# jianglab/helicon

Measured on NVIDIA B200. Metric: denovo3D candidates/sec (solve+score), higher is better.
Workload: dtype f32 (u,v,h) / f64 (x,hbar; bounded branch), as scipy executes it

## Files before the change

helicon_b200/csrc/hb2_api.cu:

```cuda
#include "../../include/helicon_b200.h"
#include "hb2_kernels.cuh"
#include "hb2_trf.cuh"
#include "hb2_symm.cuh"
#include "hb2_tie.cuh"
#include "hb2_fwd_band.cuh"
#include "hb2_adj_tile.cuh"
#include "hb2_explicit.cuh"
#include "hb2_bilinear.cuh"

#include <cub/cub.cuh>
#include <nvtx3/nvToolsExt.h>

#include <algorithm>
#include <cstdio>
#include <cstring>
#include <cstdlib>
#include <string>
#include <vector>

struct NvtxRange {
  explicit NvtxRange(const char* name) { nvtxRangePushA(name); }
  ~NvtxRange() { nvtxRangePop(); }
  NvtxRange(const NvtxRange&) = delete;
  NvtxRange& operator=(const NvtxRange&) = delete;
// ... 1626 lines not shown
  b->created = true;
  return HB2_OK;
}

extern "C" int hb2_batch_set_pixel_masks(hb2_batch* b, int32_t n_masks, const uint8_t* masks, const int32_t* cand_mask) {
  if (!b || n_masks < 0 || (n_masks > 0 && !masks) || !cand_mask) return fail(HB2_ERR_ARG, "bad argument");
  if (!b->created) return fail(HB2_ERR_STATE, "hb2_batch_set_pixel_masks must follow hb2_batch_create");
  BD& B = b->B;
  CK(cudaSetDevice(b->P->device));
  cudaStream_t st = b->stream;
  const int nc = B.nc;
  const size_t npx = (size_t)B.L2 * B.D2;
  for (int c = 0; c < nc; ++c)
    if (cand_mask[c] >= n_masks) return fail(HB2_ERR_ARG, "cand_mask entry out of range");
  std::vector<uint8_t> hm(masks, masks + (size_t)n_masks * npx);
  std::vector<int> cm(cand_mask, cand_mask + nc);
  CK(upload(b->pool, &B.pixmask, hm, st));
  CK(upload(b->pool, &B.cand_pixmask, cm, st));
  if (n_masks == 0) B.pixmask = nullptr;
  std::vector<int> neg(nc, (int)0x80000000);
  CK(cudaMemcpyAsync(b->d_bmax, neg.data(), sizeof(int) * nc, cudaMemcpyHostToDevice, st));
  k_build_rhs<<<cdiv((long long)b->nviews * B.rows_per_view, 256), 256, 0, st>>>(B, b->P->d_pix, b->nviews, b->d_bmax);
  if (b->bilinear) k_bil_rhs<<<cdiv((long long)b->nviews * B.rows_per_view, 256), 256, 0, st>>>(B, b->P->d_pix, b->nviews, b->d_bmax);
  CKL();
  CK(cudaStreamSynchronize(st));
  return HB2_OK;
}

extern "C" void hb2_batch_destroy(hb2_batch* b) {
  if (!b) return;
  cudaSetDevice(b->P->device);
  cudaStreamSynchronize(b->stream);
  b->pool.free_all();
  for (cudaEvent_t e : b->ev_pool) cudaEventDestroy(e);
  if (b->side) { cudaStreamSynchronize(b->side); cudaStreamDestroy(b->side); }
  if (b->ev_fork) cudaEventDestroy(b->ev_fork);
  if (b->ev_join) cudaEventDestroy(b->ev_join);
  if (b->h_nactive) cudaFreeHost(b->h_nactive);
  delete b;
}

static int sym_ref_order(hb2_batch* b, int c, std::vector<int>& ord) {
  const int m = b->h_msym[c];
  ord.resize(m);
  for (int r = 0; r < m; ++r) ord[r] = r;
  if (m == 0 || !b->d_sym_g) return HB2_OK;
  std::vector<int> gref(m);
  CK(cudaMemcpyAsync(gref.data(), b->d_sym_g + b->h_symoff[c], sizeof(int) * m, cudaMemcpyDeviceToHost, b->stream));
  CK(cudaStreamSynchronize(b->stream));
  int start = 0;
  for (size_t rd = 0; rd < b->h_sym_round_end.size() && start < m; ++rd) {
    const int end = std::min(m, b->h_sym_round_end[rd][c]);
    if (end > start) std::sort(ord.begin() + start, ord.begin() + end, [&](int x, int y) { return gref[x] < gref[y]; });
    start = std::max(start, end);
  }
  return HB2_OK;
}

extern "C" int hb2_batch_sym_order(hb2_batch* b, int32_t c, int32_t* ord_host, int64_t capacity) {
  if (!b || !b->created || !ord_host || c < 0 || c >= b->B.nc) return fail(HB2_ERR_ARG, "bad argument");
  if (capacity < b->h_msym[c]) return fail(HB2_ERR_ARG, "capacity too small");
  CK(cudaSetDevice(b->P->device));
  std::vector<int> ord;
  if (int e = sym_ref_order(b, c, ord)) return e;
  memcpy(ord_host, ord.data(), sizeof(int) * ord.size());
  return HB2_OK;
}

extern "C" int hb2_batch_sym_rows(hb2_batch* b, int32_t c, int32_t* n_rows, int32_t* a_host, int32_t* b_host, int64_t capacity) {
  if (!b || !b->created || c < 0 || c >= b->B.nc) return fail(HB2_ERR_ARG, "bad argument");
  CK(cudaSetDevice(b->P->device));
  int m = b->h_msym[c];
  if (n_rows) *n_rows = m;
  if (a_host && b_host) {
    if (capacity < m) return fail(HB2_ERR_ARG, "capacity too small");
    CK(cudaMemcpyAsync(a_host, b->d_sym_a + b->h_symoff[c], sizeof(int) * m, cudaMemcpyDeviceToHost, b->stream));
    CK(cudaMemcpyAsync(b_host, b->d_sym_b + b->h_symoff[c], sizeof(int) * m, cudaMemcpyDeviceToHost, b->stream));
    const int L3P = b->B.L3P, nd = b->B.ndisk;
    const std::vector<int>& i2r = b->P->int2ref;
    std::vector<int> ord;
    if (int e = sym_ref_order(b, c, ord)) return e;
    std::vector<int> ta(a_host, a_host + m), tb(b_host, b_host + m);
    for (int r = 0; r < m; ++r) {
      a_host[r] = (ta[ord[r]] % L3P) * nd + i2r[ta[ord[r]] / L3P];
      b_host[r] = (tb[ord[r]] % L3P) * nd + i2r[tb[ord[r]] / L3P];
    }
  }
  return HB2_OK;
}

extern "C" int64_t hb2_batch_rows_padded(hb2_batch* b, int32_t c, int64_t* n_data_padded) {
  if (!b || !b->created || c < 0 || c >= b->B.nc) return fail(HB2_ERR_ARG, "bad argument");
  if (n_data_padded) *n_data_padded = b->h_mdata[c];
  return (int64_t)b->h_mdata[c] + b->h_msym[c];
}

extern "C" int hb2_batch_rhs(hb2_batch* b, int32_t c, float* out) {
  if (!b || !b->created || !out || c < 0 || c >= b->B.nc) return fail(HB2_ERR_ARG, "bad argument");
  CK(cudaSetDevice(b->P->device));
  CK(cudaMemcpyAsync(out, b->B.b + b->h_uoff[c], sizeof(float) * b->h_mdata[c], cudaMemcpyDeviceToHost, b->stream));
  CK(cudaStreamSynchronize(b->stream));
  return HB2_OK;
}

enum { KC_FWD_DATA = 0, KC_FWD_SYM = 1, KC_ADJ = 2, KC_UPDATE = 3, KC_SCALAR = 4, KC_NORM = 5, KC_N = 6 };
struct ProfScope {
  hb2_batch* b;
  cudaStream_t s;
  int first = 0;
  ProfScope(hb2_batch* b_, int cls, cudaStream_t s_ = nullptr) : b(b_), s(s_ ? s_ : b_->stream) {
    if (!b->profiling) return;
    while (b->ev_pool.size() < b->ev_next + 2) { cudaEvent_t e; cudaEventCreate(&e); b->ev_pool.push_back(e); }
    first = (int)b->ev_next;
    b->ev_used.push_back({cls, first});
    cudaEventRecord(b->ev_pool[first], s);
    b->ev_next += 2;
  }
  ~ProfScope() {
    if (!b->profiling) return;
    cudaEventRecord(b->ev_pool[first + 1], s);
  }
};

static void launch_fwd_data(hb2_batch* b, int mode) {
  ProfScope ps(b, KC_FWD_DATA);
  const BD& B = b->B;
  cudaStream_t st = b->stream;
  if (b->nviews == 0) return;
  if (b->n_tie_views > 0) {
    const float* src = mode == MODE_LSMR ? B.v : B.xs;
    if (b->bilinear) {
      const dim3 gv(b->n_tie_views, B.fwd_ppv);
#define FBIL(I, Q) k_fwd_bil<I, Q, float, false><<<gv, HB2_BLOCK, 0, st>>>(B, TD{}, src, B.u, mode)
#define FBILQ(I) do { if (B.L3P == 4) FBIL(I, 1); else if (B.L3P == 8) FBIL(I, 2); else if (B.L3P == 12) FBIL(I, 3); else FBIL(I, 4); } while (0)
      if (b->idx16) FBILQ(uint16_t); else FBILQ(uint32_t);
#undef FBILQ
#undef FBIL
      k_fwd_lsym<float, false><<<gv, HB2_BLOCK, 0, st>>>(B, TD{}, src, B.u, mode);
      b->extra_launches += 1;
    } else if (b->explicit_rows) k_fwd_csr<float, false><<<dim3(b->n_tie_views, B.fwd_ppv), HB2_BLOCK, 0, st>>>(B, TD{}, src, B.u, mode);
    else if (b->idx16) k_fwd_tie<uint16_t, float, false><<<dim3(b->n_tie_views, B.fwd_ppv), HB2_BLOCK, 0, st>>>(B, TD{}, src, B.u, mode);
    else k_fwd_tie<uint32_t, float, false><<<dim3(b->n_tie_views, B.fwd_ppv), HB2_BLOCK, 0, st>>>(B, TD{}, src, B.u, mode);
    b->extra_launches += 1;
  }
  if (B.fwd_band) {
    const size_t sm = b->fwd_band_smem;
    const dim3 gb(B.bt32.nband, B.nc), gr(b->max_views, B.nc);
#define FWB(Q)                                                                                            \
  do {                                                                                                    \
    hb2_allow_big_smem((const void*)k_fwd_band<Q, float, false>);                                         \
    k_fwd_band<Q, float, false><<<gb, HB2_FWDB_THREADS, sm, st>>>(B, TD{}, nullptr, mode);                \
    k_fwd_band_reduce<Q, float, false><<<gr, HB2_BLOCK, 0, st>>>(B, TD{}, nullptr, mode);                 \
  } while (0)
    if (B.L3P == 4) FWB(1); else if (B.L3P == 8) FWB(2); else if (B.L3P == 12) FWB(3); else FWB(4);
    b->extra_launches += 1;
#undef FWB
    return;
  }
  const int ntiles = (B.D2 + HB2_TILE_RAYS - 1) / HB2_TILE_RAYS;
  unsigned grid = (unsigned)b->nviews * ntiles;
#define FWD(T)                                                                              \
  do {                                                                                      \
    if (B.L3P == 4) k_fwd_data<T, 1><<<grid, HB2_BLOCK, 0, st>>>(B, mode);                  \
    else if (B.L3P == 8) k_fwd_data<T, 2><<<grid, HB2_BLOCK, 0, st>>>(B, mode);             \
    else if (B.L3P == 12) k_fwd_data<T, 3><<<grid, HB2_BLOCK, 0, st>>>(B, mode);            \
    else k_fwd_data<T, 4><<<grid, HB2_BLOCK, 0, st>>>(B, mode);                             \
  } while (0)
  if (b->idx16) FWD(uint16_t); else FWD(uint32_t);
#undef FWD
}
static void launch_fwd_sym(hb2_batch* b, int mode, cudaStream_t on = nullptr) {
  ProfScope ps(b, KC_FWD_SYM, on);
  const BD& B = b->B;
  dim3 g(B.part_us_per_cand, B.nc);
  k_fwd_sym<<<g, HB2_BLOCK, 0, on ? on : b->stream>>>(B, mode);
}
static void launch_adj(hb2_batch* b, int mode) {
  ProfScope ps(b, KC_ADJ);
  const BD& B = b->B;
  dim3 g(B.part_v_per_cand, B.nc);
  cudaStream_t st = b->stream;
  if (b->n_tie_views > 0) {
    if (b->bilinear) {
      const dim3 ga(cdiv(B.ndisk, (HB2_BLOCK / 32) * (32 / (B.L3P / 4))), B.nc);
      const size_t smt = (size_t)HB2_BILT_NS * HB2_BILT_SV * ((size_t)B.bil_KB * HB2_BLOCK * 6 + (size_t)B.bil_rmax * B.L3P * sizeof(float));
      const bool use_tile = B.bil_adj_tile && smt <= 200 * 1024;
#define ABIL(Q)                                                                                      \
  do {                                                                                               \
    k_bil_unblend<Q, float, false><<<b->n_tie_views, HB2_BLOCK, 0, st>>>(B, TD{}, B.u, B.bil_ub, mode); \
    if (use_tile && B.bil_KB == 3) {                                                                 \
      hb2_allow_big_smem((const void*)k_adj_bil_tile<Q, 3, float, false>);                           \
      k_adj_bil_tile<Q, 3, float, false><<<dim3(B.ntile, B.nc), HB2_BILT_THREADS, smt, st>>>(B, TD{}, B.bil_ub, B.vtie, mode); \
    } else if (use_tile) {                                                                           \
      hb2_allow_big_smem((const void*)k_adj_bil_tile<Q, 0, float, false>);                           \
      k_adj_bil_tile<Q, 0, float, false><<<dim3(B.ntile, B.nc), HB2_BILT_THREADS, smt, st>>>(B, TD{}, B.bil_ub, B.vtie, mode); \
    } else k_adj_bil<Q, float, false><<<ga, HB2_BLOCK, 0, st>>>(B, TD{}, B.bil_ub, B.vtie, mode);   \
  } while (0)
      if (B.L3P == 4) ABIL(1); else if (B.L3P == 8) ABIL(2); else if (B.L3P == 12) ABIL(3); else ABIL(4);
#undef ABIL
      k_adj_lsym<float, false><<<dim3(cdiv(B.npad, HB2_BLOCK), B.nc), HB2_BLOCK, 0, st>>>(B, TD{}, B.u, B.vtie, mode);
      b->extra_launches += 2;
    } else if (b->explicit_rows) k_adj_csc<float, false><<<dim3(cdiv(B.npad, HB2_BLOCK / 32), B.nc), HB2_BLOCK, 0, st>>>(B, TD{}, B.u, B.vtie, mode);
    else k_adj_tie<float, false><<<dim3(cdiv(B.ndisk, HB2_BLOCK), B.nc), HB2_BLOCK, 0, st>>>(B, TD{}, B.u, B.vtie, mode);
    b->extra_launches += 1;
  }
  if (B.adj_tile == 2) {
    const size_t sm = b->adj_tile_smem;
    const dim3 gc(B.ntile, B.nc, b->adj_chunks);
#define ADJTC(K)                                                                                                        \
  do {                                                                                                                  \
    hb2_allow_big_smem((const void*)k_adj_tile<4, K, float, false, true>);   \
    k_adj_tile<4, K, float, false, true><<<gc, HB2_ADJT_THREADS, sm, st>>>(B, TD{}, B.u, nullptr, mode);                \
  } while (0)
    if (B.K == 1) ADJTC(1); else ADJTC(2);
#undef ADJTC
    return;
  }
  if (B.adj_tile) {
    const size_t sm = b->adj_tile_smem;
#define ADJT(Q, K)                                                                                                   \
  do {                                                                                                               \
    hb2_allow_big_smem((const void*)k_adj_tile<Q, K, float, false>);      \
    k_adj_tile<Q, K, float, false><<<g, HB2_ADJT_THREADS, sm, st>>>(B, TD{}, B.u, nullptr, mode);                    \
  } while (0)
#define ADJTQ(K) do { if (B.L3P == 4) ADJT(1, K); else if (B.L3P == 8) ADJT(2, K); else if (B.L3P == 12) ADJT(3, K); else ADJT(4, K); } while (0)
    if (B.K == 1) ADJTQ(1); else ADJTQ(2);
#undef ADJTQ
#undef ADJT
    return;
  }
  if (B.adj_fast) {
    if (B.K == 1) k_adj_pq<1><<<g, HB2_BLOCK, 0, st>>>(B, mode);
    else k_adj_pq<2><<<g, HB2_BLOCK, 0, st>>>(B, mode);
    return;
  }
#define ADJ(K, M) k_adj<K, M><<<g, HB2_BLOCK, 0, st>>>(B, mode)
  if (B.MC == 1) ADJ(0, 1);
  else ADJ(0, 0);
#undef ADJ
}
static void launch_update(hb2_batch* b, int mode) {
  ProfScope ps(b, KC_UPDATE);
  const BD& B = b->B;
  dim3 g(B.part_x_per_cand, B.nc);
  k_update<<<g, HB2_BLOCK, 0, b->stream>>>(B, mode);
}

extern "C" int hb2_batch_apply_forward(hb2_batch* b, int32_t c, const float* x_host, float* y_host) {
  if (!b || !b->created || !x_host || !y_host || c < 0 || c >= b->B.nc) return fail(HB2_ERR_ARG, "bad argument");
  CK(cudaSetDevice(b->P->device));
  BD& B = b->B;
  cudaStream_t st = b->stream;
  long long m = (long long)b->h_mdata[c] + b->h_msym[c];
  std::vector<float> xi((size_t)B.npad, 0.f);
  for (int z = 0; z < B.L3; ++z)
    for (int pp = 0; pp < B.ndisk; ++pp) xi[(size_t)pp * B.L3P + z] = x_host[(size_t)z * B.ndisk + b->P->int2ref[pp]];
  CK(cudaMemcpyAsync(B.xs + (size_t)c * B.npad, xi.data(), sizeof(float) * B.npad, cudaMemcpyHostToDevice, st));
  CK(cudaMemsetAsync(B.u + b->h_uoff[c], 0, sizeof(float) * m, st));
  B.only_cand = c;
  launch_fwd_data(b, MODE_PLAIN);
  launch_fwd_sym(b, MODE_PLAIN);
  B.only_cand = -1;
  CKL();
  CK(cudaMemcpyAsync(y_host, B.u + b->h_uoff[c], sizeof(float) * m, cudaMemcpyDeviceToHost, st));
  CK(cudaStreamSynchronize(st));
  b->solved = false;
  return HB2_OK;
}

extern "C" int hb2_batch_apply_adjoint(hb2_batch* b, int32_t c, const float* y_host, float* x_host) {
  if (!b || !b->created || !x_host || !y_host || c < 0 || c >= b->B.nc) return fail(HB2_ERR_ARG, "bad argument");
  CK(cudaSetDevice(b->P->device));
  BD& B = b->B;
  cudaStream_t st = b->stream;
  long long m = (long long)b->h_mdata[c] + b->h_msym[c];
  CK(cudaMemcpyAsync(B.u + b->h_uoff[c], y_host, sizeof(float) * m, cudaMemcpyHostToDevice, st));
  B.only_cand = c;
  launch_adj(b, MODE_PLAIN);
  B.only_cand = -1;
  CKL();
  std::vector<float> xi((size_t)B.npad);
  CK(cudaMemcpyAsync(xi.data(), B.xs + (size_t)c * B.npad, sizeof(float) * B.npad, cudaMemcpyDeviceToHost, st));
  CK(cudaStreamSynchronize(st));
  for (int z = 0; z < B.L3; ++z)
    for (int pp = 0; pp < B.ndisk; ++pp) x_host[(size_t)z * B.ndisk + b->P->int2ref[pp]] = xi[(size_t)pp * B.L3P + z];
  b->solved = false;
  return HB2_OK;
}


static int run_trf(hb2_batch* b, const hb2_solve_options* opt, std::vector<TrfState>& out, long long& launches, int& outer_iters) {
  BD& B = b->B;
  cudaStream_t st = b->stream;
  const int nc = B.nc;
  bool any = false;
  for (int c = 0; c < nc; ++c) any = any || b->cands[c].positive;
  out.assign(nc, TrfState{});
  if (!any) return HB2_OK;
  DevPool tmp;
  tmp.owner = b;
  TD T{};
#define CKT2(call) do { cudaError_t e_ = (call); if (e_ != cudaSuccess) { tmp.free_all(); return fail(HB2_ERR_CUDA, std::string(#call) + ": " + cudaGetErrorString(e_)); } } while (0)
  const size_t nv = (size_t)nc * B.npad, nu = (size_t)b->u_total;
  double** nvecs[] = {&T.G, &T.D, &T.DH, &T.PH, &T.RH, &T.STEP, &T.V, &T.H, &T.HBAR, &T.XIN, &T.W, &T.UN};
  for (double** p : nvecs) CKT2(tmp.alloc(p, nv, true, st));
  B.vtie64 = nullptr;
  if (b->n_tie_views > 0) CKT2(tmp.alloc(&B.vtie64, nv, true, st));
  B.bil_ub64 = nullptr;
  if (b->bilinear) CKT2(tmp.alloc(&B.bil_ub64, nu, true, st));
  double** mvecs[] = {&T.R, &T.UM, &T.Y, &T.Y2};
  for (double** p : mvecs) CKT2(tmp.alloc(p, nu, true, st));
  long long max_m = 0;
  for (int c = 0; c < nc; ++c) max_m = std::max<long long>(max_m, (long long)b->h_mdata[c] + b->h_msym[c]);
  const unsigned gn = cdiv(B.npad, HB2_BLOCK * 4), gm = std::max(1u, cdiv(max_m, HB2_BLOCK * 4));
  T.red_slots = (int)std::max(gn, gm);
  CKT2(tmp.alloc(&T.red, (size_t)nc * T.red_slots * TRF_NRED, true, st));
  CKT2(tmp.alloc(&T.st, nc, true, st));
  CKT2(tmp.alloc(&T.nactive, 1, true, st));
  CKT2(tmp.alloc(&T.ninner, 1, true, st));
  {
    std::vector<float> bmax(nc);
    CKT2(cudaMemcpyAsync(bmax.data(), b->d_bmax, sizeof(float) * nc, cudaMemcpyDeviceToHost, st));
    CKT2(cudaStreamSynchronize(st));
    std::vector<TrfState> hs(nc, TrfState{});
    for (int c = 0; c < nc; ++c) {
      int iv;
      memcpy(&iv, &bmax[c], 4);
      iv = iv >= 0 ? iv : iv ^ 0x7fffffff;
      float ub;
      memcpy(&ub, &iv, 4);
      hs[c].needed = b->cands[c].positive ? 1 : 0;
      hs[c].lb = 0.0; hs[c].ub = (double)ub;
      hs[c].tol = opt->trf_tol > 0 ? opt->trf_tol : 1e-2;
      if (!(hs[c].ub > hs[c].lb)) hs[c].needed = 0;
    }
    CKT2(cudaMemcpyAsync(T.st, hs.data(), sizeof(TrfState) * nc, cudaMemcpyHostToDevice, st));
    CKT2(cudaStreamSynchronize(st));
  }
  const double EPS = 2.220446049250313e-16;
  const int lsmr_maxiter = opt->max_iter > 0 ? opt->max_iter : 1000;
  const int max_iter = opt->trf_max_iter > 0 ? opt->trf_max_iter : 200;
  const dim3 g_n(gn, nc), g_m(gm, nc), g_sym(std::max(1, B.part_us_per_cand), nc);
  const dim3 g_adj(cdiv((long long)B.ndisk * (B.L3P / 4), HB2_BLOCK), nc);
  const size_t sm64 = (size_t)HB2_ADJT_NS * HB2_ADJT_SV * B.K * HB2_BLOCK * sizeof(uint16_t) +
                      (size_t)HB2_ADJT_NS * HB2_ADJT_SV * B.rmax * B.L3P * sizeof(double);
  const unsigned g_fwd = (unsigned)b->nviews * ((B.D2 + HB2_TILE_RAYS - 1) / HB2_TILE_RAYS);
  const unsigned g_sc = cdiv(nc, 128);
  auto ew = [&](int op) { k_trf_ew<<<g_n, HB2_BLOCK, 0, st>>>(B, T, op); ++launches; };
  auto mw = [&](int op) { k_trf_mw<<<g_m, HB2_BLOCK, 0, st>>>(B, T, op); ++launches; };
  auto red = [&](int nslots, int add, int gate, int start = 0) { k_trf_reduce<<<nc, HB2_BLOCK, 0, st>>>(B, T, nslots, add, gate, start); ++launches; };
  auto sc = [&](int op) { k_trf_scal<<<g_sc, 128, 0, st>>>(B, T, op, EPS, lsmr_maxiter, max_iter); ++launches; };
  auto fwd = [&](const double* src, double* dst, int gate) {
    if (B.bt64.nband > 0) {
      const dim3 gb(B.bt64.nband, nc), gr(b->max_views, nc);
#define FWB64(Q)                                                                                          \
  do {                                                                                                    \
    hb2_allow_big_smem((const void*)k_fwd_band<Q, double, true>);                                         \
    k_fwd_band<Q, double, true><<<gb, HB2_FWDB_THREADS, b->fwd_band_smem64, st>>>(B, T, src, gate);       \
    k_fwd_band_reduce<Q, double, true><<<gr, HB2_BLOCK, 0, st>>>(B, T, dst, gate);                        \
  } while (0)
      if (B.L3P == 4) FWB64(2); else if (B.L3P == 8) FWB64(4); else if (B.L3P == 12) FWB64(6); else FWB64(8);
#undef FWB64
      ++launches;
    } else if (b->idx16) k_fwd64_data<uint16_t><<<g_fwd, HB2_BLOCK, 0, st>>>(B, T, src, dst, gate);
    else k_fwd64_data<uint32_t><<<g_fwd, HB2_BLOCK, 0, st>>>(B, T, src, dst, gate);
    k_fwd64_sym<<<g_sym, HB2_BLOCK, 0, st>>>(B, T, src, dst, gate);
    launches += 2;
    if (b->n_tie_views > 0) {
      if (b->bilinear) {
        const dim3 gv(b->n_tie_views, B.fwd_ppv);
#define FBIL(I, Q) k_fwd_bil<I, Q, double, true><<<gv, HB2_BLOCK, 0, st>>>(B, T, src, dst, gate)
#define FBILQ(I) do { if (B.L3P == 4) FBIL(I, 1); else if (B.L3P == 8) FBIL(I, 2); else if (B.L3P == 12) FBIL(I, 3); else FBIL(I, 4); } while (0)
        if (b->idx16) FBILQ(uint16_t); else FBILQ(uint32_t);
#undef FBILQ
#undef FBIL
        k_fwd_lsym<double, true><<<gv, HB2_BLOCK, 0, st>>>(B, T, src, dst, gate);
        ++launches;
      } else if (b->explicit_rows) k_fwd_csr<double, true><<<dim3(b->n_tie_views, B.fwd_ppv), HB2_BLOCK, 0, st>>>(B, T, src, dst, gate);
      else if (b->idx16) k_fwd_tie<uint16_t, double, true><<<dim3(b->n_tie_views, B.fwd_ppv), HB2_BLOCK, 0, st>>>(B, T, src, dst, gate);
      else k_fwd_tie<uint32_t, double, true><<<dim3(b->n_tie_views, B.fwd_ppv), HB2_BLOCK, 0, st>>>(B, T, src, dst, gate);
      ++launches;
    }
  };
  auto adj = [&](const double* rows, double* dst, int gate) {
    if (b->n_tie_views > 0) {
      if (b->bilinear) {
        const dim3 ga(cdiv(B.ndisk, (HB2_BLOCK / 32) * (32 / (B.L3P / 4))), nc);
        const size_t smt = (size_t)HB2_BILT_NS * HB2_BILT_SV * ((size_t)B.bil_KB * HB2_BLOCK * 6 + (size_t)B.bil_rmax * B.L3P * sizeof(double));
        const bool use_tile = B.bil_adj_tile && smt <= 200 * 1024;
#define ABIL(Q)                                                                                        \
  do {                                                                                                 \
    k_bil_unblend<Q, double, true><<<b->n_tie_views, HB2_BLOCK, 0, st>>>(B, T, rows, B.bil_ub64, gate); \
    if (use_tile) {                                                                                    \
      hb2_allow_big_smem((const void*)k_adj_bil_tile<Q, 0, double, true>);                             \
      k_adj_bil_tile<Q, 0, double, true><<<dim3(B.ntile, nc), HB2_BILT_THREADS, smt, st>>>(B, T, B.bil_ub64, B.vtie64, gate); \
    } else k_adj_bil<Q, double, true><<<ga, HB2_BLOCK, 0, st>>>(B, T, B.bil_ub64, B.vtie64, gate);    \
  } while (0)
        if (B.L3P == 4) ABIL(1); else if (B.L3P == 8) ABIL(2); else if (B.L3P == 12) ABIL(3); else ABIL(4);
#undef ABIL
        k_adj_lsym<double, true><<<dim3(cdiv(B.npad, HB2_BLOCK), nc), HB2_BLOCK, 0, st>>>(B, T, rows, B.vtie64, gate);
        launches += 2;
      } else if (b->explicit_rows) k_adj_csc<double, true><<<dim3(cdiv(B.npad, HB2_BLOCK / 32), nc), HB2_BLOCK, 0, st>>>(B, T, rows, B.vtie64, gate);
      else k_adj_tie<double, true><<<dim3(cdiv(B.ndisk, HB2_BLOCK), nc), HB2_BLOCK, 0, st>>>(B, T, rows, B.vtie64, gate);
      ++launches;
    }
    if (B.adj_tile == 1 && sm64 <= 200 * 1024) {
      const dim3 gt(B.ntile, nc);
#define ADJT64(Q, K)                                                                                                 \
  do {                                                                                                               \
    hb2_allow_big_smem((const void*)k_adj_tile<Q, K, double, true>);    \
    k_adj_tile<Q, K, double, true><<<gt, HB2_ADJT_THREADS, sm64, st>>>(B, T, rows, dst, gate);                       \
  } while (0)
#define ADJT64Q(K) do { if (B.L3P == 4) ADJT64(1, K); else if (B.L3P == 8) ADJT64(2, K); else if (B.L3P == 12) ADJT64(3, K); else ADJT64(4, K); } while (0)
      if (B.K == 1) ADJT64Q(1); else ADJT64Q(2);
#undef ADJT64Q
#undef ADJT64
    } else {
      k_adj64<<<g_adj, HB2_BLOCK, 0, st>>>(B, T, rows, dst, gate);
    }
    ++launches;
  };
  auto read_counter = [&](int* dptr, int& v) -> cudaError_t {
    cudaError_t e = cudaMemcpyAsync(b->h_nactive, dptr, sizeof(int), cudaMemcpyDeviceToHost, st);
    if (e != cudaSuccess) return e;
    e = cudaStreamSynchronize(st);
    v = *b->h_nactive;
    return e;
  };
  ew(EW_START); red(gn, 0, 0, 1); sc(SC_START);
  int nact = 0;
  CKT2(read_counter(T.nactive, nact));
  outer_iters = 0;
  if (nact > 0) {
    k_trf_start_apply<<<g_n, HB2_BLOCK, 0, st>>>(B, T); ++launches;
    fwd(T.W, T.Y, 0); mw(MW_RESID); red(gm, 0, 0); sc(SC_RESID0);
    adj(T.R, T.G, 0);
    for (int it = 0; it <= max_iter && nact > 0; ++it) {
      ew(EW_PREP); red(gn, 0, 0); sc(SC_PREP);
      CKT2(read_counter(T.nactive, nact));
      if (nact == 0) break;
      ++outer_iters;
      CKT2(cudaMemsetAsync(T.ninner, 0, sizeof(int), st));
      adj(T.UM, T.W, 0); ew(EW_INNER_INIT); red(gn, 0, 0); sc(SC_INNER_INIT);
      ew(EW_INNER_UPD);
      int ninner = 1;
      for (int k = 0; k < lsmr_maxiter && ninner > 0; ++k) {
        fwd(T.W, T.Y, 1); mw(MW_INNER_U); red(gm, 0, 1);
        ew(EW_INNER_UN); red(gn, 1, 1); sc(SC_INNER_BETA);
        adj(T.UM, T.W, 1); ew(EW_INNER_V); red(gn, 0, 1); sc(SC_INNER_ROT);
        ew(EW_INNER_UPD); red(gn, 0, 1); sc(SC_INNER_TEST);
        if (k % 2 == 1 || k + 1 == lsmr_maxiter) CKT2(read_counter(T.ninner, ninner));
      }
      ew(EW_STEP1); red(gn, 0, 0); sc(SC_STEP1);
      ew(EW_STEP2); red(gn, 0, 2); sc(SC_STEP2);
      fwd(T.W, T.Y, 2);
      ew(EW_LOAD_PH); fwd(T.W, T.Y2, 2);
      mw(MW_DOTS3); red(gm, 0, 2); sc(SC_SAVE_M);
      ew(EW_DOTS); red(gn, 0, 2); sc(SC_QUAD);
      ew(EW_AG); red(gn, 0, 2); sc(SC_SAVE_AG);
      fwd(T.W, T.Y, 2); mw(MW_DOT_YY); red(gm, 0, 2); sc(SC_AG);
      ew(EW_MKSTEP); red(gn, 0, 0); sc(SC_SAVE_SG);
      fwd(T.W, T.Y, 0); mw(MW_DOT_YY); red(gm, 0, 0); sc(SC_CC);
      ew(EW_XUPD);
      fwd(T.W, T.Y, 0); mw(MW_RESID); red(gm, 0, 0); sc(SC_RESID);
      adj(T.R, T.G, 0);
      CKT2(cudaGetLastError());
    }
  }
  ew(EW_FINAL);
  CKT2(cudaGetLastError());
  CKT2(cudaMemcpyAsync(out.data(), T.st, sizeof(TrfState) * nc, cudaMemcpyDeviceToHost, st));
  CKT2(cudaStreamSynchronize(st));
  tmp.free_all();
  B.vtie64 = nullptr;
  return HB2_OK;
}

extern "C" int hb2_batch_solve(hb2_batch* b, const hb2_solve_options* opt, hb2_result* res) {
  if (!b || !b->created || !opt || !res) return fail(HB2_ERR_ARG, "bad argument");
  CK(cudaSetDevice(b->P->device));
  NvtxRange nvtx_("solve_equations + score (batch)");
  nvtxRangePushA("solve_equations: LSMR");
  struct PopGuard { int n = 1; ~PopGuard() { while (n-- > 0) nvtxRangePop(); } } nvtx_stage_;
  BD& B = b->B;
  cudaStream_t st = b->stream;
  const int nc = B.nc;
  const int maxit = opt->max_iter > 0 ? opt->max_iter : 1000;
  const int check = opt->check_every > 0 ? opt->check_every : 8;
  B.clip_pred = opt->clip_pred;
  B.only_cand = -1;
  b->profiling = opt->profile != 0;
  b->ev_used.clear();
  b->ev_next = 0;
  cudaEvent_t e0, e1, e2;
  CK(cudaEventCreate(&e0)); CK(cudaEventCreate(&e1)); CK(cudaEventCreate(&e2));
  CK(cudaEventRecord(e0, st));
  size_t nv = (size_t)nc * B.npad;
  CK(cudaMemsetAsync(B.x, 0, nv * sizeof(double), st));
  CK(cudaMemsetAsync(B.hbar, 0, nv * sizeof(double), st));
  CK(cudaMemsetAsync(B.h, 0, nv * sizeof(float), st));
  CK(cudaMemsetAsync(B.v, 0, nv * sizeof(float), st));
  CK(cudaMemcpyAsync(B.u, B.b, sizeof(float) * (size_t)b->u_total, cudaMemcpyDeviceToDevice, st));
  CK(cudaMemsetAsync(b->d_nactive, 0, sizeof(int), st));
  long long launches = 0;
  b->extra_launches = 0;
  static const int env_norm = [] { const char* e = getenv("HB2_NORM_MODE"); return e ? atoi(e) : -1; }();
  const bool chain = (env_norm >= 0 ? env_norm : opt->norm_mode) != 0;
  if (chain) {
    hb2_allow_big_smem((const void*)k_chain_sumsq<CHAIN_U>);
    hb2_allow_big_smem((const void*)k_chain_sumsq<CHAIN_V>);
    hb2_allow_big_smem((const void*)k_chain_sumsq<CHAIN_B>);
  }
  float* ch_u = chain ? b->d_chain : nullptr;
  float* ch_v = chain ? b->d_chain + nc : nullptr;
  if (chain) { k_chain_sumsq<CHAIN_B><<<nc, 64, HB2_CHAIN_SMEM, st>>>(B, ch_u, MODE_INIT); ++launches; }
  k_scal_normb<<<nc, HB2_BLOCK, 0, st>>>(B, ch_u);
  launch_adj(b, MODE_INIT);
  if (chain) { k_chain_sumsq<CHAIN_V><<<nc, 64, HB2_CHAIN_SMEM, st>>>(B, ch_v, MODE_INIT); ++launches; }
  k_scal_init<<<nc, HB2_BLOCK, 0, st>>>(B, b->d_nactive, ch_v);
  launch_update(b, MODE_INIT);
  launches += 4;
  CKL();
  int it = 0;
  static const int env_overlap = [] { const char* e = getenv("HB2_OVERLAP"); return e ? atoi(e) : 1; }();
  const bool overlap = env_overlap != 0 && !b->profiling;
  if (overlap && !b->side) {
    CK(cudaStreamCreateWithFlags(&b->side, cudaStreamNonBlocking));
    CK(cudaEventCreateWithFlags(&b->ev_fork, cudaEventDisableTiming));
    CK(cudaEventCreateWithFlags(&b->ev_join, cudaEventDisableTiming));
  }
  *b->h_nactive = 1;
  CK(cudaMemcpyAsync(b->h_nactive, b->d_nactive, sizeof(int), cudaMemcpyDeviceToHost, st));
  CK(cudaStreamSynchronize(st));
  while (*b->h_nactive > 0 && it < maxit) {
    int burst = std::min(check, maxit - it);
    for (int q = 0; q < burst; ++q) {
      if (overlap) {
        cudaEventRecord(b->ev_fork, st);
        launch_fwd_data(b, MODE_LSMR);
        cudaStreamWaitEvent(b->side, b->ev_fork, 0);
        launch_fwd_sym(b, MODE_LSMR, b->side);
        cudaEventRecord(b->ev_join, b->side);
        cudaStreamWaitEvent(st, b->ev_join, 0);
      } else {
        launch_fwd_data(b, MODE_LSMR);
        launch_fwd_sym(b, MODE_LSMR);
      }
      if (chain) { ProfScope ps(b, KC_NORM); k_chain_sumsq<CHAIN_U><<<nc, 64, HB2_CHAIN_SMEM, st>>>(B, ch_u, MODE_LSMR); ++launches; }
      { ProfScope ps(b, KC_SCALAR); k_scal_beta<<<nc, HB2_BLOCK, 0, st>>>(B, ch_u); }
      launch_adj(b, MODE_LSMR);
      if (chain) { ProfScope ps(b, KC_NORM); k_chain_sumsq<CHAIN_V><<<nc, 64, HB2_CHAIN_SMEM, st>>>(B, ch_v, MODE_LSMR); ++launches; }
      { ProfScope ps(b, KC_SCALAR); k_scal_rot<<<nc, HB2_BLOCK, 0, st>>>(B, ch_v); }
      launch_update(b, MODE_LSMR);
      { ProfScope ps(b, KC_SCALAR); k_scal_test<<<nc, HB2_BLOCK, 0, st>>>(B, opt->atol, opt->btol, opt->conlim, maxit, opt->fixed_iters, b->d_nactive); }
      launches += 7;
    }
    it += burst;
    CKL();
    CK(cudaMemcpyAsync(b->h_nactive, b->d_nactive, sizeof(int), cudaMemcpyDeviceToHost, st));
    CK(cudaStreamSynchronize(st));
  }
  CK(cudaEventRecord(e1, st));
  std::vector<TrfState> trf;
  int trf_outer = 0;
  cudaEvent_t e1b;
  CK(cudaEventCreate(&e1b));
  {
    dim3 g(cdiv(B.npad, 256), nc);
    k_x_to_f32<<<g, 256, 0, st>>>(B);
    ++launches;
  }
  nvtxRangePop(); nvtxRangePushA("solve_equations: bounded TRF");
  if (opt->fixed_iters <= 0) {
    int rc = run_trf(b, opt, trf, launches, trf_outer);
    if (rc != HB2_OK) return rc;
  } else trf.assign(nc, TrfState{});
  CK(cudaEventRecord(e1b, st));
  nvtxRangePop(); nvtxRangePushA("cosine_similarity (reprojection + score)");
  {
    launch_fwd_data(b, MODE_SCORE);
    k_scal_score<<<nc, HB2_BLOCK, 0, st>>>(B, b->d_score);
    launches += 2;
    CKL();
  }
  CK(cudaEventRecord(e2, st));
  std::vector<LsmrState> hs(nc);
  std::vector<float> sc(nc);
  CK(cudaMemcpyAsync(hs.data(), B.st, sizeof(LsmrState) * nc, cudaMemcpyDeviceToHost, st));
  CK(cudaMemcpyAsync(sc.data(), b->d_score, sizeof(float) * nc, cudaMemcpyDeviceToHost, st));
  CK(cudaStreamSynchronize(st));
  float ms_l = 0, ms_s = 0, ms_t = 0;
  cudaEventElapsedTime(&ms_l, e0, e1); cudaEventElapsedTime(&ms_t, e1, e1b); cudaEventElapsedTime(&ms_s, e1b, e2);
  cudaEventDestroy(e0); cudaEventDestroy(e1); cudaEventDestroy(e1b); cudaEventDestroy(e2);
  for (double& t : b->timing) t = 0;
  b->timing[0] = ms_l; b->timing[1] = ms_t; b->timing[2] = ms_s; b->timing[13] = trf_outer; b->timing[3] = (double)(launches + b->extra_launches); b->timing[4] = it;
  if (b->profiling) {
    for (auto& pr : b->ev_used) {
      float ms = 0;
      cudaEventElapsedTime(&ms, b->ev_pool[pr.second], b->ev_pool[pr.second + 1]);
      if (pr.first == KC_NORM) b->timing[14] += ms;
      else b->timing[5 + pr.first] += ms;
      if (pr.first == KC_FWD_DATA) b->timing[10] += 1;
      if (pr.first == KC_ADJ) b->timing[11] += 1;
      if (pr.first == KC_UPDATE) b->timing[12] += 1;
    }
    b->profiling = false;
  }
  for (int c = 0; c < nc; ++c) {
    hb2_result& r = res[c];
    r.score = sc[c]; r.itn = hs[c].itn; r.istop = hs[c].istop; r.trf_nit = trf[c].status == 3 ? 0 : trf[c].nit;
    r.flags = b->cand_flags[c] | ((trf[c].needed && trf[c].status != 3) ? HB2_FLAG_BOUNDED : 0u);
    r.n_data_rows = 0; r.n_sym_rows = b->h_msym[c];
    r.normr = (float)hs[c].normr; r.normar = hs[c].normar; r.normA = (float)hs[c].normA; r.normx = (float)hs[c].normx;
  }
  b->solved = true;
  b->last_trf = trf;
  return HB2_OK;
}

extern "C" int hb2_batch_trf_trace(hb2_batch* b, int32_t c, double* out, int32_t max_rows) {
  if (!b || !out || c < 0 || c >= (int)b->last_trf.size()) return fail(HB2_ERR_ARG, "bad argument or no solve yet");
  const TrfState& S = b->last_trf[c];
  int n = std::min(std::min(S.nit, 24), (int)max_rows);
  for (int i = 0; i < n; ++i)
    for (int k = 0; k < 8; ++k) out[i * 8 + k] = S.trace[i][k];
  return S.nit * 16 + (S.status + 1);
}

extern "C" int hb2_batch_get_x(hb2_batch* b, int32_t c, float* x_host) {
  if (!b || !b->solved || !x_host || c < 0 || c >= b->B.nc) return fail(HB2_ERR_ARG, "bad argument or batch not solved");
  CK(cudaSetDevice(b->P->device));
  const BD& B = b->B;
  std::vector<float> xi((size_t)B.npad);
  CK(cudaMemcpyAsync(xi.data(), B.xs + (size_t)c * B.npad, sizeof(float) * B.npad, cudaMemcpyDeviceToHost, b->stream));
  CK(cudaStreamSynchronize(b->stream));
  for (int z = 0; z < B.L3; ++z)
    for (int pp = 0; pp < B.ndisk; ++pp) x_host[(size_t)z * B.ndisk + b->P->int2ref[pp]] = xi[(size_t)pp * B.L3P + z];
  return HB2_OK;
}

extern "C" int hb2_batch_timing(hb2_batch* b, double* out16) {
  if (!b || !out16) return fail(HB2_ERR_ARG, "null argument");
  memcpy(out16, b->timing, sizeof(b->timing));
  return HB2_OK;
}

extern "C" int hb2_lsmr_scalar_step(double* state64, int phase, float alpha, float beta, double normx, double atol,
                                    double btol, double conlim, int maxiter, float* coef_hbar, float* coef_x,
                                    float* coef_h, double* trace8) {
  static_assert(sizeof(LsmrState) <= 64 * sizeof(double), "state scratch too small");
  LsmrState S;
  memcpy(&S, state64, sizeof(S));
  int ret = 0;
  if (phase == 0) lsmr_init_(S, alpha, beta);
  else if (phase == 1) lsmr_rotate_(S, alpha, beta);
  else ret = lsmr_test_(S, normx, atol, btol, conlim, maxiter);
  memcpy(state64, &S, sizeof(S));
  if (coef_hbar) *coef_hbar = S.cf_hbar;
  if (coef_x) *coef_x = S.cf_x;
  if (coef_h) *coef_h = S.cf_h;
  if (trace8) {
    trace8[0] = S.rho; trace8[1] = S.rhobar; trace8[2] = S.zeta; trace8[3] = S.normr; trace8[4] = S.normA;
    trace8[5] = S.test1; trace8[6] = S.test2; trace8[7] = S.active;
  }
  return ret;
}

extern "C" int hb2_helical_symmetrize(const float* data_host, const hb2_symm_params* p, const int64_t* k_begin,
                                      const int32_t* ent_h, const int32_t* ent_floor, const int32_t* ent_ceil,
                                      const double* ent_wk, const double* mats, int32_t n_mats, float* vol_out_host,
                                      float* xsum_out, float* ysum_out, float* zsum_out, int device, void* stream) {
  NvtxRange nvtx_("apply_helical_symmetry");
  if (!data_host || !p || !k_begin || !mats) return fail(HB2_ERR_ARG, "null argument");
  if (hb2_device_count() <= 0) return fail(HB2_ERR_NO_DEVICE, "no CUDA device visible; helicon_b200 has no CPU fallback");
  if (p->nz1 <= 0 || p->ny1 <= 0 || p->nx1 <= 0 || p->csym <= 0 || p->n_ent < 0) return fail(HB2_ERR_ARG, "bad sizes");
  if (p->zs0 < 0 || p->zs1 > p->nz1) return fail(HB2_ERR_ARG, "z-section slab outside the output");
  CK(cudaSetDevice(device));
  cudaStream_t st = (cudaStream_t)stream;
  SymmP P{};
  P.nz0 = p->nz0; P.ny0 = p->ny0; P.nx0 = p->nx0; P.nz = p->nz; P.ny = p->ny; P.nx = p->nx;
  P.oz = p->oz; P.oy = p->oy; P.ox = p->ox; P.nz1 = p->nz1; P.ny1 = p->ny1; P.nx1 = p->nx1;
  P.apix = p->apix; P.new_apix = p->new_apix; P.csym = p->csym; P.zs0 = p->zs0; P.zs1 = p->zs1;
  for (int e = 0; e < p->n_ent; ++e)
    if (ent_floor[e] < 0 || ent_ceil[e] >= p->nz0 || ent_h[e] < 0 || (long long)(ent_h[e] + 1) * p->csym > n_mats)
      return fail(HB2_ERR_ARG, "entry table out of range");
  DevPool pool;
  const size_t nd = (size_t)p->nz0 * p->ny0 * p->nx0, nv = (size_t)p->nz1 * p->ny1 * p->nx1;
  float *d_data, *d_vol, *d_x, *d_y, *d_z;
  long long* d_kb; int *d_h, *d_f, *d_c; double *d_w, *d_m;
#define CKS(call) do { cudaError_t e_ = (call); if (e_ != cudaSuccess) { pool.free_all(); return fail(HB2_ERR_CUDA, std::string(#call) + ": " + cudaGetErrorString(e_)); } } while (0)
  CKS(pool.alloc(&d_data, nd, false, st)); CKS(pool.alloc(&d_vol, nv, false, st));
  CKS(pool.alloc(&d_x, (size_t)p->nz1 * p->ny1, false, st)); CKS(pool.alloc(&d_y, (size_t)p->nz1 * p->nx1, false, st));
  CKS(pool.alloc(&d_z, (size_t)p->ny1 * p->nx1, false, st));
  CKS(pool.alloc(&d_kb, (size_t)p->nz1 + 1, false, st)); CKS(pool.alloc(&d_h, (size_t)p->n_ent, false, st));
  CKS(pool.alloc(&d_f, (size_t)p->n_ent, false, st)); CKS(pool.alloc(&d_c, (size_t)p->n_ent, false, st));
  CKS(pool.alloc(&d_w, (size_t)p->n_ent, false, st)); CKS(pool.alloc(&d_m, (size_t)n_mats * 4, false, st));
  CKS(cudaMemcpyAsync(d_data, data_host, nd * sizeof(float), cudaMemcpyHostToDevice, st));
  CKS(cudaMemcpyAsync(d_kb, k_begin, ((size_t)p->nz1 + 1) * sizeof(long long), cudaMemcpyHostToDevice, st));
  if (p->n_ent) {
    CKS(cudaMemcpyAsync(d_h, ent_h, (size_t)p->n_ent * sizeof(int), cudaMemcpyHostToDevice, st));
    CKS(cudaMemcpyAsync(d_f, ent_floor, (size_t)p->n_ent * sizeof(int), cudaMemcpyHostToDevice, st));
    CKS(cudaMemcpyAsync(d_c, ent_ceil, (size_t)p->n_ent * sizeof(int), cudaMemcpyHostToDevice, st));
    CKS(cudaMemcpyAsync(d_w, ent_wk, (size_t)p->n_ent * sizeof(double), cudaMemcpyHostToDevice, st));
  }
  CKS(cudaMemcpyAsync(d_m, mats, (size_t)n_mats * 4 * sizeof(double), cudaMemcpyHostToDevice, st));
  k_symm_volume<<<cdiv((long long)nv, 256), 256, 0, st>>>(P, d_data, d_kb, d_h, d_f, d_c, d_w, d_m, d_vol);
  const long long nproj = (long long)p->nz1 * p->ny1 + (long long)p->nz1 * p->nx1 + (long long)p->ny1 * p->nx1;
  k_symm_project<<<cdiv(nproj, 128), 128, 0, st>>>(P, d_vol, d_x, d_y, d_z);
  CKS(cudaGetLastError());
  if (vol_out_host) CKS(cudaMemcpyAsync(vol_out_host, d_vol, nv * sizeof(float), cudaMemcpyDeviceToHost, st));
  if (xsum_out) CKS(cudaMemcpyAsync(xsum_out, d_x, (size_t)p->nz1 * p->ny1 * sizeof(float), cudaMemcpyDeviceToHost, st));
  if (ysum_out) CKS(cudaMemcpyAsync(ysum_out, d_y, (size_t)p->nz1 * p->nx1 * sizeof(float), cudaMemcpyDeviceToHost, st));
  if (zsum_out) CKS(cudaMemcpyAsync(zsum_out, d_z, (size_t)p->ny1 * p->nx1 * sizeof(float), cudaMemcpyDeviceToHost, st));
  CKS(cudaStreamSynchronize(st));
  pool.free_all();
#undef CKS
  return HB2_OK;
}

struct hb2_scoremap {
  int device = 0;
  long long n = 0;
  float* d_score = nullptr;
  int* d_itn = nullptr;
  unsigned* d_flags = nullptr;
  long long* d_idx = nullptr;
  size_t idx_cap = 0;
  float* d_top = nullptr;
  long long* d_topi = nullptr;
  int top_cap = 0;
};

__global__ void k_scoremap_fill(float* __restrict__ sc, int* __restrict__ it, unsigned* __restrict__ fl, long long n) {
  const long long i = (long long)blockIdx.x * blockDim.x + threadIdx.x;
  if (i < n) { sc[i] = __int_as_float(0x7fc00000); it[i] = 0; fl[i] = 0u; }
}
__global__ void k_scoremap_scatter(const float* __restrict__ score, const LsmrState* __restrict__ st,
                                   const long long* __restrict__ idx, int nc, long long n, float* __restrict__ sc,
                                   int* __restrict__ it, unsigned* __restrict__ fl) {
  const int c = blockIdx.x * blockDim.x + threadIdx.x;
  if (c >= nc) return;
  const long long t = idx[c];
  if (t < 0 || t >= n) return;
  sc[t] = score[c];
  it[t] = st[c].itn;
  fl[t] = (unsigned)idx[nc + c];
}
__global__ void k_scoremap_merge(float* __restrict__ sc, int* __restrict__ it, unsigned* __restrict__ fl,
                                 const float* __restrict__ g, int n_maps, long long n) {
  const long long i = (long long)blockIdx.x * blockDim.x + threadIdx.x;
  if (i >= n) return;
  float s = sc[i];
  int q = it[i];
  unsigned f = fl[i];
  for (int r = 0; r < n_maps; ++r) {
    const float v = g[(size_t)r * 3 * n + i];
    if (v == v && !(s == s)) {
      s = v;
      q = reinterpret_cast<const int*>(g)[(size_t)r * 3 * n + n + i];
      f = reinterpret_cast<const unsigned*>(g)[(size_t)r * 3 * n + 2 * n + i];
    }
  }
  sc[i] = s; it[i] = q; fl[i] = f;
}
__global__ void __launch_bounds__(1024) k_scoremap_topk(const float* __restrict__ sc, long long n, int k,
                                                        float* __restrict__ top, long long* __restrict__ topi) {
  __shared__ float s_v[32];
  __shared__ long long s_i[32];
  __shared__ float prev_v;
  __shared__ long long prev_i;
  if (threadIdx.x == 0) { prev_v = INFINITY; prev_i = -1; }
  __syncthreads();
// ... 156 lines not shown
```

helicon_b200/csrc/hb2_trf.cuh:

```cuda
#pragma once
#include "hb2_kernels.cuh"

#define TRF_NRED 8

struct Lsmr64 {
  double alpha, beta, normb;
  double zetabar, alphabar, rho, rhobar, cbar, sbar;
  double betadd, betad, rhodold, tautildeold, thetatilde, zeta, d;
  double normA2, maxrbar, minrbar, normA, normr, normar, normx, condA, rhotemp;
  double cf_hbar, cf_x, cf_h, inv_alpha, inv_beta;
  int minrbar_inf, itn, istop, active, skip_adj;
};

struct TrfState {
  double lb, ub, tol;
  double cost, g_norm, theta, lsmr_tol, p_dot_g, p_stride, r_stride_u, r_stride_l, r_stride, ag_stride;
  double cost_change;
  double coef_p, coef_r, coef_ag;
  double acc[TRF_NRED];
  double m0, m1, m2, r_value, p_value, ag_n0, ag_n1, ag_min, step_g;
  int active;
  int needed;
  int status, nit, stop_next, full_step;
  Lsmr64 in;
  double ag_value;
  double trace[24][8];
};

struct TD {
  TrfState* st;
  double *G, *D, *DH, *PH, *RH, *STEP, *V, *H, *HBAR, *XIN, *W, *UN;
  double *R, *UM, *Y, *Y2;
  double* red;
  int red_slots;
  int* nactive;
  int* ninner;
};

HB2_HD void sym_ortho64_(double a, double b, double& c, double& s, double& r) {
  if (b == 0.0) { c = a > 0 ? 1.0 : (a < 0 ? -1.0 : 0.0); s = 0.0; r = fabs(a); }
  else if (a == 0.0) { c = 0.0; s = b > 0 ? 1.0 : -1.0; r = fabs(b); }
  else if (fabs(b) > fabs(a)) { double tau = a / b; s = (b > 0 ? 1.0 : -1.0) / sqrt(1 + tau * tau); c = s * tau; r = b / s; }
  else { double tau = b / a; c = (a > 0 ? 1.0 : -1.0) / sqrt(1 + tau * tau); s = c * tau; r = a / c; }
}
HB2_HD void lsmr64_init_(Lsmr64& S, double alpha, double beta) {
  S.alpha = alpha; S.beta = beta; S.normb = beta;
  S.zetabar = alpha * beta; S.alphabar = alpha; S.rho = 1; S.rhobar = 1; S.cbar = 1; S.sbar = 0;
  S.betadd = beta; S.betad = 0; S.rhodold = 1; S.tautildeold = 0; S.thetatilde = 0; S.zeta = 0; S.d = 0;
  S.normA2 = alpha * alpha; S.maxrbar = 0; S.minrbar = 0; S.minrbar_inf = 1; S.normA = sqrt(S.normA2);
  S.condA = 1; S.normx = 0; S.normr = beta; S.normar = alpha * beta; S.itn = 0; S.istop = 0; S.skip_adj = 0;
  S.cf_hbar = S.cf_x = S.cf_h = 0; S.rhotemp = 0;
  S.inv_alpha = alpha > 0 ? 1.0 / alpha : 1.0;
  S.inv_beta = beta > 0 ? 1.0 / beta : 0.0;
  S.active = (S.normar != 0.0 && beta != 0.0) ? 1 : 0;
}
HB2_HD void lsmr64_rotate_(Lsmr64& S, double alpha, double beta) {
  S.itn += 1; S.alpha = alpha; S.beta = beta;
  double chat = S.alphabar > 0 ? 1.0 : (S.alphabar < 0 ? -1.0 : 0.0), alphahat = fabs(S.alphabar);
  double rhoold = S.rho, c, s;
  sym_ortho64_(alphahat, beta, c, s, S.rho);
  double thetanew = s * alpha;
  S.alphabar = c * alpha;
  double rhobarold = S.rhobar, zetaold = S.zeta, thetabar = S.sbar * S.rho;
  S.rhotemp = S.cbar * S.rho;
  double cb, sb, rb;
  sym_ortho64_(S.cbar * S.rho, thetanew, cb, sb, rb);
  S.cbar = cb; S.sbar = sb; S.rhobar = rb;
  S.zeta = S.cbar * S.zetabar; S.zetabar = -S.sbar * S.zetabar;
  S.cf_hbar = -(thetabar * S.rho / (rhoold * rhobarold));
  S.cf_x = S.zeta / (S.rho * S.rhobar);
  S.cf_h = -(thetanew / S.rho);
  double betaacute = chat * S.betadd, betahat = c * betaacute;
  S.betadd = -s * betaacute;
  double thetatildeold = S.thetatilde, ct, st, rt;
  sym_ortho64_(S.rhodold, thetabar, ct, st, rt);
  S.thetatilde = st * S.rhobar; S.rhodold = ct * S.rhobar;
  S.betad = -st * S.betad + ct * betahat;
  S.tautildeold = (zetaold - thetatildeold * S.tautildeold) / rt;
  double taud = (S.zeta - S.thetatilde * S.tautildeold) / S.rhodold;
  S.normr = sqrt(S.d + (S.betad - taud) * (S.betad - taud) + S.betadd * S.betadd);
  S.normA2 += beta * beta; S.normA = sqrt(S.normA2); S.normA2 += alpha * alpha;
  S.maxrbar = fmax(S.maxrbar, rhobarold);
  if (S.itn > 1) { S.minrbar = S.minrbar_inf ? rhobarold : fmin(S.minrbar, rhobarold); S.minrbar_inf = 0; }
  double mn = S.minrbar_inf ? S.rhotemp : fmin(S.minrbar, S.rhotemp);
  S.condA = fmax(S.maxrbar, S.rhotemp) / mn;
  S.normar = fabs(S.zetabar);
  S.inv_alpha = alpha > 0 ? 1.0 / alpha : 1.0;
}
HB2_HD int lsmr64_test_(Lsmr64& S, double normx, double atol, double btol, double conlim, int maxiter) {
  S.normx = normx;
  double test1 = S.normr / S.normb;
  double test2 = (S.normA * S.normr) != 0 ? S.normar / (S.normA * S.normr) : INFINITY;
  double test3 = 1 / S.condA;
  double t1 = test1 / (1 + S.normA * normx / S.normb);
  double rtol = btol + atol * S.normA * normx / S.normb;
  double ctol = conlim > 0 ? 1 / conlim : 0;
  int istop = 0;
  if (S.itn >= maxiter) istop = 7;
  if (1 + test3 <= 1) istop = 6;
  if (1 + test2 <= 1) istop = 5;
  if (1 + t1 <= 1) istop = 4;
  if (test3 <= ctol) istop = 3;
  if (test2 <= atol) istop = 2;
  if (test1 <= rtol) istop = 1;
  S.istop = istop;
  return istop;
}

__device__ __forceinline__ bool trf_gate(const TrfState& S, int gate) {
  if (!S.active) return false;
  if (gate == 1) return S.in.active != 0;
  if (gate == 2) return S.full_step == 0;
  return true;
}

template <typename IdxT>
__global__ void __launch_bounds__(HB2_BLOCK) k_fwd64_data(BD B, TD T, const double* __restrict__ src, double* __restrict__ dst,
                                                         int inner) {
  const int ntiles = (B.D2 + HB2_TILE_RAYS - 1) / HB2_TILE_RAYS;
  const int view = blockIdx.x / ntiles, tile = blockIdx.x % ntiles;
  const int c = B.view_cand[view];
  if (B.view_tie && B.view_tie[view] >= 0) return;
  const TrfState& S = T.st[c];
  if (!trf_gate(S, inner)) return;
  __shared__ int s_colk[HB2_MAX_ZMC];
  for (int e = threadIdx.x; e < B.ZMC; e += HB2_BLOCK) s_colk[e] = B.colk[B.view_colbegin[view] + e];
  __syncthreads();
  const int a = B.view_angle[view];
  const int D2 = B.D2, L3 = B.L3, L3P = B.L3P, MC = B.MC, ZMP = B.ZMP;
  const IdxT* __restrict__ fm = (const IdxT*)B.fmap + (size_t)a * D2 * D2;
  const double* __restrict__ vsrc = src + (size_t)c * B.npad;
  double* urow = dst + B.view_uoff[view];
  const int warp = threadIdx.x >> 5, lane = threadIdx.x & 31;
  const int q = lane & 3, sg = lane >> 2;
  const uint8_t* __restrict__ pm = cand_mask(B, c);
  for (int r = warp; r < HB2_TILE_RAYS; r += HB2_BLOCK / 32) {
    const int j = tile * HB2_TILE_RAYS + r;
    if (j >= D2) break;
    if (!B.rayvalid[a * D2 + j]) continue;
    const IdxT* __restrict__ fj = fm + (size_t)j * D2;
    for (int z0 = 0; z0 < L3P; z0 += 16) {
      double acc[4] = {0, 0, 0, 0};
      const int zq = z0 + 4 * q;
      if (zq < L3P) {
        const double* __restrict__ vb = vsrc + zq;
        for (int i0 = sg; i0 < D2; i0 += 32) {
          IdxT ids[4];
#pragma unroll
          for (int w = 0; w < 4; ++w) ids[w] = (i0 + 8 * w < D2) ? fj[i0 + 8 * w] : Sent<IdxT>::v;
          double2 ta[4], tb[4];
#pragma unroll
          for (int w = 0; w < 4; ++w) {
            if (ids[w] != Sent<IdxT>::v) {
              const double2* vp = reinterpret_cast<const double2*>(vb + (size_t)ids[w] * L3P);
              ta[w] = __ldg(vp); tb[w] = __ldg(vp + 1);
            } else {
              ta[w] = make_double2(0.0, 0.0); tb[w] = make_double2(0.0, 0.0);
            }
          }
#pragma unroll
          for (int w = 0; w < 4; ++w)
            if (ids[w] != Sent<IdxT>::v) { acc[0] += ta[w].x; acc[1] += ta[w].y; acc[2] += tb[w].x; acc[3] += tb[w].y; }
        }
      }
#pragma unroll
      for (int o = 4; o < 32; o <<= 1)
#pragma unroll
        for (int t = 0; t < 4; ++t) acc[t] += __shfl_xor_sync(0xffffffffu, acc[t], o);
      if (sg < 4) {
        const int z = zq + sg;
        if (z < L3) {
          const double sum = sg == 0 ? acc[0] : (sg == 1 ? acc[1] : (sg == 2 ? acc[2] : acc[3]));
          for (int mc = 0; mc < MC; ++mc) {
            const int zm = z * MC + mc;
            if (s_colk[zm] >= 0 && !(pm && !pm[(size_t)s_colk[zm] * D2 + j])) urow[(size_t)j * ZMP + zm] = sum;
          }
        }
      }
    }
  }
}

__global__ void __launch_bounds__(HB2_BLOCK) k_fwd64_sym(BD B, TD T, const double* __restrict__ src, double* __restrict__ dst,
                                                        int inner) {
  const int c = blockIdx.y;
  const TrfState& S = T.st[c];
  if (!trf_gate(S, inner)) return;
  const int m = B.cand_msym[c];
  const double* __restrict__ vsrc = src + (size_t)c * B.npad;
  double* us = dst + B.cand_uoff[c] + B.cand_mdata[c];
  const int* __restrict__ sa = B.sym_a + B.cand_symoff[c];
  const int* __restrict__ sb = B.sym_b + B.cand_symoff[c];
  for (int r = blockIdx.x * HB2_BLOCK * 4 + threadIdx.x, qq = 0; qq < 4; ++qq, r += HB2_BLOCK)
    if (r < m) us[r] = __ldg(vsrc + sa[r]) - __ldg(vsrc + sb[r]);
}

__global__ void __launch_bounds__(HB2_BLOCK) k_adj64(BD B, TD T, const double* __restrict__ rows, double* __restrict__ dst,
                                                    int inner) {
  const int c = blockIdx.y;
  const TrfState& S = T.st[c];
  if (!trf_gate(S, inner) || (inner == 1 && S.in.skip_adj)) return;
  const int L3 = B.L3, L3P = B.L3P, ZMP = B.ZMP, ndisk = B.ndisk, K = B.K, MC = B.MC;
  const int NQ = L3P >> 2;
  const int t = blockIdx.x * HB2_BLOCK + threadIdx.x;
  const int p = t / NQ, q = t - p * NQ;
  if (p >= ndisk) return;
  const int slot = B.aslot[p];
  const int z0 = 4 * q;
  double acc[4] = {0.0, 0.0, 0.0, 0.0};
  const int vb = B.cand_view_begin[c], nv = B.cand_view_count[c];
  for (int vi = 0; vi < nv; ++vi) {
    const int view = vb + vi;
    if (B.view_tie && B.view_tie[view] >= 0) continue;
    const int a = __ldg(B.view_angle + view);
    const double* __restrict__ ub = rows + __ldg(B.view_uoff + view) + z0 * MC;
    const uint16_t* __restrict__ am = B.amap + (size_t)a * K * B.apitch + slot;
    for (int k = 0; k < K; ++k) {
      const uint16_t j = am[(size_t)k * B.apitch];
      if (j != 0xFFFFu) {
        const double* __restrict__ uj = ub + (size_t)j * ZMP;
        if (MC == 1) {
          const double2 r0 = __ldg(reinterpret_cast<const double2*>(uj));
          const double2 r1 = __ldg(reinterpret_cast<const double2*>(uj) + 1);
          acc[0] += r0.x; acc[1] += r0.y; acc[2] += r1.x; acc[3] += r1.y;
        } else {
#pragma unroll
          for (int zz = 0; zz < 4; ++zz)
            if (z0 + zz < L3)
              for (int mc = 0; mc < MC; ++mc) acc[zz] += __ldg(uj + zz * MC + mc);
        }
      }
    }
  }
  const int* __restrict__ ptr = B.csc_ptr + (size_t)c * (B.npad + 1);
  const int* __restrict__ ent = B.csc_ent + B.cand_cscoff[c];
  const double* __restrict__ us = rows + B.cand_uoff[c] + B.cand_mdata[c];
  double* vdst = dst + (size_t)c * B.npad + (size_t)p * L3P + z0;
  if (B.vtie64 && B.cand_tie_count[c] > 0) {
    const double* vt = B.vtie64 + (size_t)c * B.npad + (size_t)p * L3P + z0;
#pragma unroll
    for (int zz = 0; zz < 4; ++zz) acc[zz] += vt[zz];
  }
#pragma unroll
  for (int zz = 0; zz < 4; ++zz) {
    double a2 = acc[zz];
    if (z0 + zz < L3) {
      const int g = p * L3P + z0 + zz;
      for (int e = ptr[g]; e < ptr[g + 1]; ++e) {
        int en = ent[e];
        double val = __ldg(us + (en & 0x7fffffff));
        a2 += en < 0 ? -val : val;
      }
    }
    vdst[zz] = a2;
  }
}

__device__ __forceinline__ double block_minmax_d(double x, bool is_min, double* shd) {
#pragma unroll
  for (int o = 16; o > 0; o >>= 1) {
    double y = __shfl_xor_sync(0xffffffffu, x, o);
    x = is_min ? fmin(x, y) : fmax(x, y);
  }
  int w = threadIdx.x >> 5, l = threadIdx.x & 31;
  if (l == 0) shd[w] = x;
  __syncthreads();
  if (w == 0) {
    x = l < HB2_BLOCK / 32 ? shd[l] : (is_min ? INFINITY : -INFINITY);
#pragma unroll
    for (int o = 16; o > 0; o >>= 1) {
      double y = __shfl_xor_sync(0xffffffffu, x, o);
      x = is_min ? fmin(x, y) : fmax(x, y);
    }
  }
  __syncthreads();
  return x;
}
__device__ __forceinline__ void trf_store_partials(TD T, int c, int slot, double (&v)[TRF_NRED], double* shd) {
#pragma unroll
  for (int k = 0; k < TRF_NRED; ++k) {
    double x = k < 6 ? block_sum_d(v[k], shd) : block_minmax_d(v[k], k == 6, shd);
    if (threadIdx.x == 0) T.red[((size_t)c * T.red_slots + slot) * TRF_NRED + k] = x;
  }
}
__global__ void __launch_bounds__(HB2_BLOCK) k_trf_reduce(BD B, TD T, int nslots, int add, int gate, int start) {
  const int c = blockIdx.x;
  __shared__ double shd[HB2_BLOCK / 32];
  TrfState& S = T.st[c];
  if (!(start ? (S.needed != 0) : trf_gate(S, gate))) return;
  double v[TRF_NRED];
#pragma unroll
  for (int k = 0; k < TRF_NRED; ++k) v[k] = k < 6 ? 0.0 : (k == 6 ? INFINITY : -INFINITY);
  for (int s2 = threadIdx.x; s2 < nslots; s2 += HB2_BLOCK) {
    const double* p = T.red + ((size_t)c * T.red_slots + s2) * TRF_NRED;
#pragma unroll
    for (int k = 0; k < 6; ++k) v[k] += p[k];
    v[6] = fmin(v[6], p[6]); v[7] = fmax(v[7], p[7]);
  }
#pragma unroll
  for (int k = 0; k < TRF_NRED; ++k) {
    double x = k < 6 ? block_sum_d(v[k], shd) : block_minmax_d(v[k], k == 6, shd);
    if (threadIdx.x == 0) {
      if (add) S.acc[k] = k < 6 ? S.acc[k] + x : (k == 6 ? fmin(S.acc[k], x) : fmax(S.acc[k], x));
      else S.acc[k] = x;
    }
  }
}

__device__ __forceinline__ double step_to_bound(double x, double s, double lb, double ub) {
  if (s == 0.0) return INFINITY;
  return fmax((lb - x) / s, (ub - x) / s);
}

enum {
  EW_START = 0,
  EW_PREP,
  EW_INNER_INIT,
  EW_INNER_UN,
  EW_INNER_V,
  EW_INNER_UPD,
  EW_STEP1,
  EW_STEP2,
  EW_LOAD_PH,
  EW_DOTS,
  EW_AG,
  EW_MKSTEP,
  EW_XUPD,
  EW_FINAL
};

__global__ void __launch_bounds__(HB2_BLOCK) k_trf_ew(BD B, TD T, int op) {
  const int c = blockIdx.y;
  __shared__ double shd[HB2_BLOCK / 32];
  const TrfState& S = T.st[c];
  bool act;
  if (op == EW_START || op == EW_FINAL) act = S.needed != 0;
  else if (op == EW_INNER_UPD) act = S.active && (S.in.active || S.in.itn == 0);
  else if (op == EW_INNER_UN || op == EW_INNER_V) act = trf_gate(S, 1);
  else if (op == EW_STEP2 || op == EW_LOAD_PH || op == EW_DOTS || op == EW_AG) act = trf_gate(S, 2);
  else act = trf_gate(S, 0);
  if (op == EW_INNER_V && S.in.skip_adj) act = false;
  if (!act) return;
  const size_t o = (size_t)c * B.npad;
  double* X = B.x + o;
  double red[TRF_NRED] = {0, 0, 0, 0, 0, 0, INFINITY, -INFINITY};
  const double lb = S.lb, ub = S.ub;
  for (int i = blockIdx.x * HB2_BLOCK * 4 + threadIdx.x, qq = 0; qq < 4; ++qq, i += HB2_BLOCK) {
    if (i >= B.npad || (i % B.L3P) >= B.L3) continue;
    const size_t e = o + i;
    switch (op) {
      case EW_START: {
        double y = X[i];
        red[6] = fmin(red[6], y); red[7] = fmax(red[7], y);
      } break;
      case EW_PREP: {
        double x = X[i], g = T.G[e], v = 1.0, dv = 0.0;
        if (g < 0) { v = ub - x; dv = -1.0; }
        if (g > 0) { v = x - lb; dv = 1.0; }
        T.D[e] = sqrt(v); T.DH[e] = g * dv;
        red[7] = fmax(red[7], fabs(g * v));
      } break;
      case EW_INNER_INIT: {
        double vt = T.D[e] * T.W[e];
        T.UN[e] = 0.0; T.V[e] = vt; red[0] += vt * vt;
      } break;
      case EW_INNER_UN: {
        double un = sqrt(T.DH[e]) * T.V[e] - S.in.alpha * (T.UN[e] * S.in.inv_beta);
        T.UN[e] = un; red[0] += un * un;
      } break;
      case EW_INNER_V: {
        double vt = (T.D[e] * T.W[e] + sqrt(T.DH[e]) * T.UN[e]) * S.in.inv_beta - S.in.beta * T.V[e];
        T.V[e] = vt; red[0] += vt * vt;
      } break;
      case EW_INNER_UPD: {
        double vn = T.V[e];
        if (S.in.itn == 0 || !S.in.skip_adj) { vn *= S.in.inv_alpha; T.V[e] = vn; }
        if (S.in.itn == 0) { T.H[e] = vn; T.HBAR[e] = 0.0; T.XIN[e] = 0.0; }
        else {
          double ho = T.H[e];
          double hb = T.HBAR[e] * S.in.cf_hbar + ho;
          T.HBAR[e] = hb;
          double xn = T.XIN[e] + S.in.cf_x * hb;
          T.XIN[e] = xn;
          T.H[e] = ho * S.in.cf_h + vn;
          red[0] += xn * xn;
        }
        T.W[e] = T.D[e] * vn;
      } break;
      case EW_STEP1: {
        double ph = -T.XIN[e];
        T.PH[e] = ph;
        double x = X[i], p = T.D[e] * ph, xp = x + p;
        red[6] = fmin(red[6], fmin(xp - lb, ub - xp));
        red[5] += p * T.G[e];
        red[7] = fmax(red[7], -step_to_bound(x, p, lb, ub));
      } break;
      case EW_STEP2: {
        double ph = T.PH[e], x = X[i], d = T.D[e];
        double p = d * ph;
        double st = step_to_bound(x, p, lb, ub);
        double rh = (st == S.p_stride && p != 0.0) ? -ph : ph;
        T.RH[e] = rh;
        T.PH[e] = ph * S.p_stride;
        double xb = x + p * S.p_stride, r = d * rh;
        red[7] = fmax(red[7], -step_to_bound(xb, r, lb, ub));
        T.W[e] = r;
      } break;
      case EW_LOAD_PH: T.W[e] = T.D[e] * T.PH[e]; break;
      case EW_DOTS: {
        double ph = T.PH[e], rh = T.RH[e], dh = T.DH[e], gh = T.D[e] * T.G[e];
        red[0] += rh * dh * rh; red[1] += gh * rh; red[2] += ph * dh * rh; red[3] += gh * ph; red[4] += ph * dh * ph;
      } break;
      case EW_AG: {
        double d = T.D[e], g = T.G[e], gh = d * g, agh = -gh, ag = d * agh;
        red[0] += agh * T.DH[e] * agh; red[1] += gh * agh;
        red[7] = fmax(red[7], -step_to_bound(X[i], ag, lb, ub));
        T.W[e] = ag;
      } break;
      case EW_MKSTEP: {
        double d = T.D[e];
        double s2 = d * (S.coef_p * T.PH[e] + S.coef_r * T.RH[e] - S.coef_ag * (d * T.G[e]));
        T.STEP[e] = s2; T.W[e] = s2; red[0] += s2 * T.G[e];
      } break;
      case EW_XUPD: {
        double x = X[i];
        if (S.cost_change >= 0) {
          x = x + T.STEP[e];
          if (x <= lb) x = nextafter(lb, ub);
          if (x >= ub) x = nextafter(ub, lb);
          if (x < lb || x > ub) x = 0.5 * (lb + ub);
          X[i] = x;
        }
        T.W[e] = x;
      } break;
      case EW_FINAL: B.xs[e] = (float)X[i]; break;
    }
  }
  if (op == EW_LOAD_PH || op == EW_XUPD || op == EW_FINAL) return;
  trf_store_partials(T, c, blockIdx.x, red, shd);
}

__global__ void __launch_bounds__(HB2_BLOCK) k_trf_start_apply(BD B, TD T) {
  const int c = blockIdx.y;
  const TrfState& S = T.st[c];
  if (!S.active) return;
  double* X = B.x + (size_t)c * B.npad;
  const double lb = S.lb, ub = S.ub, d = ub - lb;
  for (int i = blockIdx.x * HB2_BLOCK * 4 + threadIdx.x, qq = 0; qq < 4; ++qq, i += HB2_BLOCK) {
    if (i >= B.npad || (i % B.L3P) >= B.L3) continue;
    double y = X[i];
    double t = fmod(y - lb, 2 * d);
    if (t < 0) t += 2 * d;
    double x = lb + fmin(t, 2 * d - t);
    double ld = x - lb, udist = ub - x;
    double lth = 0.1 * fmax(1.0, fabs(lb)), uth = 0.1 * fmax(1.0, fabs(ub));
    bool la = ld <= fmin(udist, lth), ua = udist <= fmin(ld, uth);
    if (la) x = lb + 0.1 * fmax(1.0, fabs(lb));
    if (ua) x = ub - 0.1 * fmax(1.0, fabs(ub));
    if (x < lb || x > ub) x = 0.5 * (lb + ub);
    X[i] = x;
    T.W[(size_t)c * B.npad + i] = x;
  }
}

enum { MW_RESID = 0, MW_INNER_U, MW_DOTS3, MW_DOT_YY };
__global__ void __launch_bounds__(HB2_BLOCK) k_trf_mw(BD B, TD T, int op) {
  const int c = blockIdx.y;
  __shared__ double shd[HB2_BLOCK / 32];
  const TrfState& S = T.st[c];
  bool act = op == MW_INNER_U ? trf_gate(S, 1) : (op == MW_DOTS3 ? trf_gate(S, 2) : trf_gate(S, 0));
  if (!act) return;
  const long long m = (long long)B.cand_mdata[c] + B.cand_msym[c];
  const size_t o = (size_t)B.cand_uoff[c];
  double red[TRF_NRED] = {0, 0, 0, 0, 0, 0, INFINITY, -INFINITY};
  for (long long r = (long long)blockIdx.x * HB2_BLOCK * 4 + threadIdx.x, qq = 0; qq < 4; ++qq, r += HB2_BLOCK) {
    if (r >= m) continue;
    const size_t e = o + r;
    switch (op) {
      case MW_RESID: {
        double bb = r < B.cand_mdata[c] ? (double)B.b[e] : 0.0;
        double res = T.Y[e] - bb;
        T.R[e] = res; T.UM[e] = res; red[0] += res * res;
      } break;
      case MW_INNER_U: {
        double un = T.Y[e] - S.in.alpha * (T.UM[e] * S.in.inv_beta);
        T.UM[e] = un; red[0] += un * un;
      } break;
      case MW_DOTS3: {
        double v1 = T.Y[e], u1 = T.Y2[e];
        red[0] += v1 * v1; red[1] += u1 * v1; red[2] += u1 * u1;
      } break;
      case MW_DOT_YY: { double v = T.Y[e]; red[0] += v * v; } break;
    }
  }
  trf_store_partials(T, c, blockIdx.x, red, shd);
}

enum {
  SC_START = 0, SC_RESID0, SC_PREP, SC_INNER_INIT, SC_INNER_BETA, SC_INNER_ROT, SC_INNER_TEST, SC_STEP1, SC_STEP2,
  SC_SAVE_M, SC_QUAD, SC_SAVE_AG, SC_AG, SC_SAVE_SG, SC_CC, SC_RESID
};
__device__ __forceinline__ void min_quadratic_1d(double a, double b, double lo, double hi, double c, double& t, double& y) {
  double tt[3] = {lo, hi, 0};
  int n = 2;
  if (a != 0) {
    double ext = -0.5 * b / a;
    if (lo < ext && ext < hi) tt[n++] = ext;
  }
  t = tt[0]; y = tt[0] * (a * tt[0] + b) + c;
  for (int k = 1; k < n; ++k) {
    double yy = tt[k] * (a * tt[k] + b) + c;
    if (yy < y) { y = yy; t = tt[k]; }
  }
}
__global__ void k_trf_scal(BD B, TD T, int op, double eps, int lsmr_maxiter, int max_iter) {
  const int c = blockIdx.x * blockDim.x + threadIdx.x;
  if (c >= B.nc) return;
  TrfState& S = T.st[c];
  if (op == SC_START) { if (!S.needed) return; }
  else if (op == SC_INNER_BETA || op == SC_INNER_ROT || op == SC_INNER_TEST) { if (!trf_gate(S, 1)) return; }
  else if (op == SC_STEP2 || op == SC_SAVE_M || op == SC_QUAD || op == SC_SAVE_AG || op == SC_AG) { if (!trf_gate(S, 2)) return; }
  else if (!trf_gate(S, 0)) return;
  const double* r = S.acc;
  switch (op) {
    case SC_START: {
      bool inb = r[6] >= S.lb && r[7] <= S.ub;
      S.active = inb ? 0 : 1; S.status = inb ? 3 : 0; S.nit = 0; S.stop_next = 0; S.full_step = 0;
      if (!inb) atomicAdd(T.nactive, 1);
    } break;
    case SC_RESID0: S.cost = 0.5 * r[0]; break;
    case SC_PREP: {
      S.g_norm = r[7];
      bool stop = S.stop_next != 0;
      if (S.g_norm < S.tol) { S.status = 1; stop = true; }
      if (!stop && S.nit >= max_iter) stop = true;
      if (stop) { S.active = 0; if (S.nit < max_iter) S.nit += 1; atomicSub(T.nactive, 1); break; }
      S.nit += 1;
      if (S.nit <= 24) { S.trace[S.nit - 1][0] = S.cost; S.trace[S.nit - 1][1] = S.g_norm; }
      double eta = 1e-2 * fmin(0.5, S.g_norm);
      S.lsmr_tol = fmax(eps, fmin(0.1, eta * S.g_norm));
      S.theta = 1 - fmin(0.005, S.g_norm);
      S.in.beta = sqrt(2 * S.cost);
      S.in.inv_beta = S.in.beta > 0 ? 1.0 / S.in.beta : 0.0;
      S.in.itn = 0; S.in.active = 1; S.in.skip_adj = 0; S.in.alpha = 0; S.full_step = 0;
    } break;
    case SC_INNER_INIT: {
      double nv = sqrt(r[0]);
      double beta = S.in.beta;
      lsmr64_init_(S.in, nv * (beta > 0 ? 1.0 / beta : 0.0), beta);
      S.in.inv_alpha = nv > 0 ? 1.0 / nv : 1.0;
      if (S.in.active) atomicAdd(T.ninner, 1);
    } break;
    case SC_INNER_BETA: {
      S.in.beta = sqrt(r[0]);
      if (S.in.beta > 0) { S.in.inv_beta = 1.0 / S.in.beta; S.in.skip_adj = 0; } else S.in.skip_adj = 1;
    } break;
    case SC_INNER_ROT: lsmr64_rotate_(S.in, S.in.skip_adj ? S.in.alpha : sqrt(r[0]), S.in.beta); break;
    case SC_INNER_TEST: {
      int istop = lsmr64_test_(S.in, sqrt(r[0]), S.lsmr_tol, S.lsmr_tol, 1e8, lsmr_maxiter);
      if (istop > 0) { S.in.active = 0; atomicSub(T.ninner, 1); }
    } break;
    case SC_STEP1: {
      S.p_dot_g = r[5];
      if (S.p_dot_g > 0) { S.status = -1; S.stop_next = 1; }
      S.full_step = r[6] >= 0.0 ? 1 : 0;
      S.p_stride = -r[7];
      if (S.full_step) { S.coef_p = 1.0; S.coef_r = 0.0; S.coef_ag = 0.0; }
    } break;
    case SC_STEP2: {
      double rsu = -r[7];
      S.r_stride_l = (1 - S.theta) * rsu;
      S.r_stride_u = rsu * S.theta;
    } break;
    case SC_SAVE_M: S.m0 = r[0]; S.m1 = r[1]; S.m2 = r[2]; break;
    case SC_QUAD: {
      double a = 0.5 * (S.m0 + r[0]);
      double b = r[1] + S.m1 + r[2];
      double cc = 0.5 * S.m2 + r[3] + 0.5 * r[4];
      if (S.r_stride_u > 0) min_quadratic_1d(a, b, S.r_stride_l, S.r_stride_u, cc, S.r_stride, S.r_value);
      else { S.r_value = INFINITY; S.r_stride = 0; }
      double th = S.theta;
      S.p_value = 0.5 * (th * th * S.m2 + th * th * r[4]) + th * r[3];
    } break;
    case SC_SAVE_AG: S.ag_n0 = r[0]; S.ag_n1 = r[1]; S.ag_min = -r[7]; break;
    case SC_AG: {
      double a = 0.5 * (r[0] + S.ag_n0), b = S.ag_n1;
      double ag_value;
      min_quadratic_1d(a, b, 0.0, S.ag_min * S.theta, 0.0, S.ag_stride, ag_value);
      S.ag_value = ag_value;
      if (S.p_value < S.r_value && S.p_value < ag_value) { S.coef_p = S.theta; S.coef_r = 0; S.coef_ag = 0; }
      else if (S.r_value < S.p_value && S.r_value < ag_value) { S.coef_p = 1.0; S.coef_r = S.r_stride; S.coef_ag = 0; }
      else { S.coef_p = 0; S.coef_r = 0; S.coef_ag = S.ag_stride; }
    } break;
    case SC_SAVE_SG: S.step_g = r[0]; break;
    case SC_CC: {
      S.cost_change = -(0.5 * r[0] + S.step_g);
      if (S.nit <= 24) {
        double* t = S.trace[S.nit - 1];
        t[2] = S.in.itn;
        t[3] = S.full_step ? 0 : (S.coef_ag != 0 ? 3 : (S.coef_r != 0 ? 2 : 1));
        t[4] = S.p_value; t[5] = S.r_value; t[6] = S.ag_value; t[7] = S.cost_change;
      }
    } break;
    case SC_RESID: {
      if (S.cost_change < S.tol * S.cost) { S.status = 2; S.stop_next = 1; }
      S.cost = 0.5 * r[0];
    } break;
  }
}
```

Before: 54.46.

## Fuse TRF elementwise, reduce and scalar kernels; batch step-selection forward passes

Replaces the separate elementwise, m-space, reduce and scalar-update kernels of the bounded TRF solver with templated per-op pass kernels and a reduce kernel that also performs the scalar state update. Several outer-iteration phases are merged so the three candidate-step forward projections (p, r, anti-gradient) run back to back into separate buffers. This removes many small launches and redundant forward and adjoint applications per iteration. Each thread now handles more elements, reductions are masked to the needed slots, and the adjoint at inner-loop initialisation is dropped. The cost is extra m-space buffers and a more intricate op/mask table that must stay numerically equivalent to the previous sequence. A profiling script is added alongside.

```diff
diff --git a/helicon_b200/csrc/hb2_api.cu b/helicon_b200/csrc/hb2_api.cu
--- a/helicon_b200/csrc/hb2_api.cu
+++ b/helicon_b200/csrc/hb2_api.cu
@@ -1952,18 +1952,20 @@
   TD T{};
 #define CKT2(call) do { cudaError_t e_ = (call); if (e_ != cudaSuccess) { tmp.free_all(); return fail(HB2_ERR_CUDA, std::string(#call) + ": " + cudaGetErrorString(e_)); } } while (0)
   const size_t nv = (size_t)nc * B.npad, nu = (size_t)b->u_total;
-  double** nvecs[] = {&T.G, &T.D, &T.DH, &T.PH, &T.RH, &T.STEP, &T.V, &T.H, &T.HBAR, &T.XIN, &T.W, &T.UN};
+  double** nvecs[] = {&T.G, &T.D, &T.DH, &T.PH, &T.RH, &T.V, &T.H, &T.HBAR, &T.XIN, &T.W, &T.UN};
   for (double** p : nvecs) CKT2(tmp.alloc(p, nv, true, st));
+  T.W2 = T.HBAR; T.AG = T.H;
   B.vtie64 = nullptr;
   if (b->n_tie_views > 0) CKT2(tmp.alloc(&B.vtie64, nv, true, st));
   B.bil_ub64 = nullptr;
   if (b->bilinear) CKT2(tmp.alloc(&B.bil_ub64, nu, true, st));
-  double** mvecs[] = {&T.R, &T.UM, &T.Y, &T.Y2};
+  double** mvecs[] = {&T.R, &T.UM, &T.Y, &T.YP, &T.YAG};
   for (double** p : mvecs) CKT2(tmp.alloc(p, nu, true, st));
   long long max_m = 0;
   for (int c = 0; c < nc; ++c) max_m = std::max<long long>(max_m, (long long)b->h_mdata[c] + b->h_msym[c]);
-  const unsigned gn = cdiv(B.npad, HB2_BLOCK * 4), gm = std::max(1u, cdiv(max_m, HB2_BLOCK * 4));
-  T.red_slots = (int)std::max(gn, gm);
+  const unsigned gn = cdiv(B.npad, TRF_SPAN), gm = std::max(1u, cdiv(max_m, TRF_SPAN));
+  T.gn = (int)gn; T.gm = (int)gm;
+  T.red_slots = (int)(gn + gm);
   CKT2(tmp.alloc(&T.red, (size_t)nc * T.red_slots * TRF_NRED, true, st));
   CKT2(tmp.alloc(&T.st, nc, true, st));
   CKT2(tmp.alloc(&T.nactive, 1, true, st));
@@ -1990,16 +1992,24 @@
   const double EPS = 2.220446049250313e-16;
   const int lsmr_maxiter = opt->max_iter > 0 ? opt->max_iter : 1000;
   const int max_iter = opt->trf_max_iter > 0 ? opt->trf_max_iter : 200;
-  const dim3 g_n(gn, nc), g_m(gm, nc), g_sym(std::max(1, B.part_us_per_cand), nc);
+  const dim3 g_sym(std::max(1, B.part_us_per_cand), nc);
   const dim3 g_adj(cdiv((long long)B.ndisk * (B.L3P / 4), HB2_BLOCK), nc);
   const size_t sm64 = (size_t)HB2_ADJT_NS * HB2_ADJT_SV * B.K * HB2_BLOCK * sizeof(uint16_t) +
                       (size_t)HB2_ADJT_NS * HB2_ADJT_SV * B.rmax * B.L3P * sizeof(double);
   const unsigned g_fwd = (unsigned)b->nviews * ((B.D2 + HB2_TILE_RAYS - 1) / HB2_TILE_RAYS);
-  const unsigned g_sc = cdiv(nc, 128);
-  auto ew = [&](int op) { k_trf_ew<<<g_n, HB2_BLOCK, 0, st>>>(B, T, op); ++launches; };
-  auto mw = [&](int op) { k_trf_mw<<<g_m, HB2_BLOCK, 0, st>>>(B, T, op); ++launches; };
-  auto red = [&](int nslots, int add, int gate, int start = 0) { k_trf_reduce<<<nc, HB2_BLOCK, 0, st>>>(B, T, nslots, add, gate, start); ++launches; };
-  auto sc = [&](int op) { k_trf_scal<<<g_sc, 128, 0, st>>>(B, T, op, EPS, lsmr_maxiter, max_iter); ++launches; };
+  auto pass = [&](auto op) {
+    constexpr int OP = decltype(op)::value;
+    k_trf_pass<OP><<<dim3(trf_blocks(OP, gn, gm), nc), HB2_BLOCK, 0, st>>>(B, T);
+    ++launches;
+  };
+  auto red = [&](auto op, int sc) {
+    constexpr int OP = decltype(op)::value;
+    k_trf_reduce<<<nc, HB2_BLOCK, 0, st>>>(B, T, (int)trf_blocks(OP, gn, gm), trf_mask(OP), sc, EPS, lsmr_maxiter, max_iter);
+    ++launches;
+  };
+  auto pr = [&](auto op, int sc) { pass(op); red(op, sc); };
+  using std::integral_constant;
+#define OPC(X) integral_constant<int, X>{}
   auto fwd = [&](const double* src, double* dst, int gate) {
     if (B.bt64.nband > 0) {
       const dim3 gb(B.bt64.nband, nc), gr(b->max_views, nc);
@@ -2077,47 +2087,41 @@
     v = *b->h_nactive;
     return e;
   };
-  ew(EW_START); red(gn, 0, 0, 1); sc(SC_START);
+  pr(OPC(EW_START), SC_START);
   int nact = 0;
   CKT2(read_counter(T.nactive, nact));
   outer_iters = 0;
   if (nact > 0) {
-    k_trf_start_apply<<<g_n, HB2_BLOCK, 0, st>>>(B, T); ++launches;
-    fwd(T.W, T.Y, 0); mw(MW_RESID); red(gm, 0, 0); sc(SC_RESID0);
+    pass(OPC(EW_START_APPLY));
+    fwd(T.W, T.Y, 0); pr(OPC(MW_RESID), SC_RESID0);
     adj(T.R, T.G, 0);
     for (int it = 0; it <= max_iter && nact > 0; ++it) {
-      ew(EW_PREP); red(gn, 0, 0); sc(SC_PREP);
+      CKT2(cudaMemsetAsync(T.ninner, 0, sizeof(int), st));
+      pr(OPC(EW_PREP), SC_PREP);
       CKT2(read_counter(T.nactive, nact));
       if (nact == 0) break;
       ++outer_iters;
-      CKT2(cudaMemsetAsync(T.ninner, 0, sizeof(int), st));
-      adj(T.UM, T.W, 0); ew(EW_INNER_INIT); red(gn, 0, 0); sc(SC_INNER_INIT);
-      ew(EW_INNER_UPD);
+      pass(OPC(EW_INNER_UPD));
       int ninner = 1;
       for (int k = 0; k < lsmr_maxiter && ninner > 0; ++k) {
-        fwd(T.W, T.Y, 1); mw(MW_INNER_U); red(gm, 0, 1);
-        ew(EW_INNER_UN); red(gn, 1, 1); sc(SC_INNER_BETA);
-        adj(T.UM, T.W, 1); ew(EW_INNER_V); red(gn, 0, 1); sc(SC_INNER_ROT);
-        ew(EW_INNER_UPD); red(gn, 0, 1); sc(SC_INNER_TEST);
+        fwd(T.W, T.Y, 1); pr(OPC(NM_INNER_U), SC_INNER_BETA);
+        adj(T.UM, T.W, 1); pr(OPC(EW_INNER_V), SC_INNER_ROT);
+        pr(OPC(EW_INNER_UPD), SC_INNER_TEST);
         if (k % 2 == 1 || k + 1 == lsmr_maxiter) CKT2(read_counter(T.ninner, ninner));
       }
-      ew(EW_STEP1); red(gn, 0, 0); sc(SC_STEP1);
-      ew(EW_STEP2); red(gn, 0, 2); sc(SC_STEP2);
-      fwd(T.W, T.Y, 2);
-      ew(EW_LOAD_PH); fwd(T.W, T.Y2, 2);
-      mw(MW_DOTS3); red(gm, 0, 2); sc(SC_SAVE_M);
-      ew(EW_DOTS); red(gn, 0, 2); sc(SC_QUAD);
-      ew(EW_AG); red(gn, 0, 2); sc(SC_SAVE_AG);
-      fwd(T.W, T.Y, 2); mw(MW_DOT_YY); red(gm, 0, 2); sc(SC_AG);
-      ew(EW_MKSTEP); red(gn, 0, 0); sc(SC_SAVE_SG);
-      fwd(T.W, T.Y, 0); mw(MW_DOT_YY); red(gm, 0, 0); sc(SC_CC);
-      ew(EW_XUPD);
-      fwd(T.W, T.Y, 0); mw(MW_RESID); red(gm, 0, 0); sc(SC_RESID);
+      pr(OPC(EW_STEP1), SC_STEP1);
+      pr(OPC(EW_STEP2), SC_STEP2);
+      fwd(T.W, T.Y, 2); fwd(T.W2, T.YP, 0); fwd(T.AG, T.YAG, 2);
+      pr(OPC(MW_DOTS), SC_SELECT);
+      pr(OPC(NM_STEP), SC_CC);
+      pass(OPC(EW_XUPD));
+      fwd(T.W, T.Y, 0); pr(OPC(MW_RESID), SC_RESID);
       adj(T.R, T.G, 0);
       CKT2(cudaGetLastError());
     }
   }
-  ew(EW_FINAL);
+  pass(OPC(EW_FINAL));
+#undef OPC
   CKT2(cudaGetLastError());
   CKT2(cudaMemcpyAsync(out.data(), T.st, sizeof(TrfState) * nc, cudaMemcpyDeviceToHost, st));
   CKT2(cudaStreamSynchronize(st));
diff --git a/helicon_b200/csrc/hb2_trf.cuh b/helicon_b200/csrc/hb2_trf.cuh
--- a/helicon_b200/csrc/hb2_trf.cuh
+++ b/helicon_b200/csrc/hb2_trf.cuh
@@ -2,6 +2,8 @@
 #include "hb2_kernels.cuh"
 
 #define TRF_NRED 8
+#define TRF_EPT 16
+#define TRF_SPAN (HB2_BLOCK * TRF_EPT)
 
 struct Lsmr64 {
   double alpha, beta, normb;
@@ -18,7 +20,8 @@
   double cost_change;
   double coef_p, coef_r, coef_ag;
   double acc[TRF_NRED];
-  double m0, m1, m2, r_value, p_value, ag_n0, ag_n1, ag_min, step_g;
+  double qn[5];
+  double r_value, p_value, ag_n0, ag_n1, ag_min;
   int active;
   int needed;
   int status, nit, stop_next, full_step;
@@ -29,10 +32,12 @@
 
 struct TD {
   TrfState* st;
-  double *G, *D, *DH, *PH, *RH, *STEP, *V, *H, *HBAR, *XIN, *W, *UN;
-  double *R, *UM, *Y, *Y2;
+  double *G, *D, *DH, *PH, *RH, *V, *H, *HBAR, *XIN, *W, *UN;
+  double *W2, *AG;
+  double *R, *UM, *Y, *YP, *YAG;
   double* red;
   int red_slots;
+  int gn, gm;
   int* nactive;
   int* ninner;
 };
@@ -256,53 +261,29 @@
   }
 }
 
-__device__ __forceinline__ double block_minmax_d(double x, bool is_min, double* shd) {
-#pragma unroll
-  for (int o = 16; o > 0; o >>= 1) {
-    double y = __shfl_xor_sync(0xffffffffu, x, o);
-    x = is_min ? fmin(x, y) : fmax(x, y);
-  }
-  int w = threadIdx.x >> 5, l = threadIdx.x & 31;
-  if (l == 0) shd[w] = x;
+__device__ __forceinline__ double trf_combine(int k, double a, double b) {
+  return k < 6 ? a + b : (k == 6 ? fmin(a, b) : fmax(a, b));
+}
+__device__ __forceinline__ double trf_identity(int k) { return k < 6 ? 0.0 : (k == 6 ? INFINITY : -INFINITY); }
+
+__device__ __forceinline__ void trf_block_reduce(double (&v)[TRF_NRED], unsigned mask, double (*shd)[HB2_BLOCK / 32]) {
+  const int w = threadIdx.x >> 5, l = threadIdx.x & 31;
+#pragma unroll
+  for (int k = 0; k < TRF_NRED; ++k) {
+    if (!(mask >> k & 1u)) continue;
+#pragma unroll
+    for (int o = 16; o > 0; o >>= 1) v[k] = trf_combine(k, v[k], __shfl_xor_sync(0xffffffffu, v[k], o));
+    if (l == 0) shd[k][w] = v[k];
+  }
   __syncthreads();
   if (w == 0) {
-    x = l < HB2_BLOCK / 32 ? shd[l] : (is_min ? INFINITY : -INFINITY);
-#pragma unroll
-    for (int o = 16; o > 0; o >>= 1) {
-      double y = __shfl_xor_sync(0xffffffffu, x, o);
-      x = is_min ? fmin(x, y) : fmax(x, y);
-    }
-  }
-  __syncthreads();
-  return x;
-}
-__device__ __forceinline__ void trf_store_partials(TD T, int c, int slot, double (&v)[TRF_NRED], double* shd) {
-#pragma unroll
-  for (int k = 0; k < TRF_NRED; ++k) {
-    double x = k < 6 ? block_sum_d(v[k], shd) : block_minmax_d(v[k], k == 6, shd);
-    if (threadIdx.x == 0) T.red[((size_t)c * T.red_slots + slot) * TRF_NRED + k] = x;
-  }
-}
-__global__ void __launch_bounds__(HB2_BLOCK) k_trf_reduce(BD B, TD T, int nslots, int add, int gate, int start) {
-  const int c = blockIdx.x;
-  __shared__ double shd[HB2_BLOCK / 32];
-  TrfState& S = T.st[c];
-  if (!(start ? (S.needed != 0) : trf_gate(S, gate))) return;
-  double v[TRF_NRED];
-#pragma unroll
-  for (int k = 0; k < TRF_NRED; ++k) v[k] = k < 6 ? 0.0 : (k == 6 ? INFINITY : -INFINITY);
-  for (int s2 = threadIdx.x; s2 < nslots; s2 += HB2_BLOCK) {
-    const double* p = T.red + ((size_t)c * T.red_slots + s2) * TRF_NRED;
-#pragma unroll
-    for (int k = 0; k < 6; ++k) v[k] += p[k];
-    v[6] = fmin(v[6], p[6]); v[7] = fmax(v[7], p[7]);
-  }
-#pragma unroll
-  for (int k = 0; k < TRF_NRED; ++k) {
-    double x = k < 6 ? block_sum_d(v[k], shd) : block_minmax_d(v[k], k == 6, shd);
-    if (threadIdx.x == 0) {
-      if (add) S.acc[k] = k < 6 ? S.acc[k] + x : (k == 6 ? fmin(S.acc[k], x) : fmax(S.acc[k], x));
-      else S.acc[k] = x;
+#pragma unroll
+    for (int k = 0; k < TRF_NRED; ++k) {
+      if (!(mask >> k & 1u)) continue;
+      double x = l < HB2_BLOCK / 32 ? shd[k][l] : trf_identity(k);
+#pragma unroll
+      for (int o = 16; o > 0; o >>= 1) x = trf_combine(k, x, __shfl_xor_sync(0xffffffffu, x, o));
+      v[k] = x;
     }
   }
 }
@@ -314,144 +295,59 @@
 
 enum {
   EW_START = 0,
+  EW_START_APPLY,
   EW_PREP,
-  EW_INNER_INIT,
-  EW_INNER_UN,
   EW_INNER_V,
   EW_INNER_UPD,
   EW_STEP1,
   EW_STEP2,
-  EW_LOAD_PH,
-  EW_DOTS,
-  EW_AG,
-  EW_MKSTEP,
   EW_XUPD,
-  EW_FINAL
+  EW_FINAL,
+  MW_RESID,
+  MW_DOTS,
+  NM_INNER_U,
+  NM_STEP
 };
-
-__global__ void __launch_bounds__(HB2_BLOCK) k_trf_ew(BD B, TD T, int op) {
-  const int c = blockIdx.y;
-  __shared__ double shd[HB2_BLOCK / 32];
-  const TrfState& S = T.st[c];
-  bool act;
-  if (op == EW_START || op == EW_FINAL) act = S.needed != 0;
-  else if (op == EW_INNER_UPD) act = S.active && (S.in.active || S.in.itn == 0);
-  else if (op == EW_INNER_UN || op == EW_INNER_V) act = trf_gate(S, 1);
-  else if (op == EW_STEP2 || op == EW_LOAD_PH || op == EW_DOTS || op == EW_AG) act = trf_gate(S, 2);
-  else act = trf_gate(S, 0);
-  if (op == EW_INNER_V && S.in.skip_adj) act = false;
-  if (!act) return;
-  const size_t o = (size_t)c * B.npad;
-  double* X = B.x + o;
-  double red[TRF_NRED] = {0, 0, 0, 0, 0, 0, INFINITY, -INFINITY};
+__host__ __device__ constexpr bool trf_has_n(int op) { return op < MW_RESID || op >= NM_INNER_U; }
+__host__ __device__ constexpr bool trf_has_m(int op) { return op >= MW_RESID; }
+__host__ __device__ constexpr unsigned trf_mask(int op) {
+  return op == EW_START ? 0xC0u : op == EW_PREP ? 0xC7u : op == EW_STEP1 ? 0xE0u : op == EW_STEP2 ? 0x9Fu
+       : op == MW_DOTS ? 0x0Fu : op == NM_STEP ? 0x03u
+       : (op == EW_START_APPLY || op == EW_XUPD || op == EW_FINAL) ? 0u : 0x01u;
+}
+__host__ __device__ constexpr unsigned trf_blocks(int op, unsigned gn, unsigned gm) {
+  return (trf_has_n(op) ? gn : 0u) + (trf_has_m(op) ? gm : 0u);
+}
+
+__device__ __forceinline__ bool trf_pass_active(const TrfState& S, int op) {
+  switch (op) {
+    case EW_START: case EW_FINAL: return S.needed != 0;
+    case EW_START_APPLY: return S.active != 0;
+    case EW_INNER_UPD: return S.active && (S.in.active || S.in.itn == 0);
+    case NM_INNER_U: return trf_gate(S, 1);
+    case EW_INNER_V: return trf_gate(S, 1) && !S.in.skip_adj;
+    case MW_DOTS: return trf_gate(S, 2);
+    default: return trf_gate(S, 0);
+  }
+}
+
+__device__ __forceinline__ double trf_step(const TrfState& S, const TD& T, size_t e) {
+  const double d = T.D[e];
+  return d * (S.coef_p * T.PH[e] + S.coef_r * T.RH[e] - S.coef_ag * (d * T.G[e]));
+}
+
+template <int OP>
+__device__ __forceinline__ void trf_n_elem(const BD& B, const TD& T, const TrfState& S, double* X, int i, size_t e,
+                                           double (&red)[TRF_NRED]) {
   const double lb = S.lb, ub = S.ub;
-  for (int i = blockIdx.x * HB2_BLOCK * 4 + threadIdx.x, qq = 0; qq < 4; ++qq, i += HB2_BLOCK) {
-    if (i >= B.npad || (i % B.L3P) >= B.L3) continue;
-    const size_t e = o + i;
-    switch (op) {
-      case EW_START: {
-        double y = X[i];
-        red[6] = fmin(red[6], y); red[7] = fmax(red[7], y);
-      } break;
-      case EW_PREP: {
-        double x = X[i], g = T.G[e], v = 1.0, dv = 0.0;
-        if (g < 0) { v = ub - x; dv = -1.0; }
-        if (g > 0) { v = x - lb; dv = 1.0; }
-        T.D[e] = sqrt(v); T.DH[e] = g * dv;
-        red[7] = fmax(red[7], fabs(g * v));
-      } break;
-      case EW_INNER_INIT: {
-        double vt = T.D[e] * T.W[e];
-        T.UN[e] = 0.0; T.V[e] = vt; red[0] += vt * vt;
-      } break;
-      case EW_INNER_UN: {
-        double un = sqrt(T.DH[e]) * T.V[e] - S.in.alpha * (T.UN[e] * S.in.inv_beta);
-        T.UN[e] = un; red[0] += un * un;
-      } break;
-      case EW_INNER_V: {
-        double vt = (T.D[e] * T.W[e] + sqrt(T.DH[e]) * T.UN[e]) * S.in.inv_beta - S.in.beta * T.V[e];
-        T.V[e] = vt; red[0] += vt * vt;
-      } break;
-      case EW_INNER_UPD: {
-        double vn = T.V[e];
-        if (S.in.itn == 0 || !S.in.skip_adj) { vn *= S.in.inv_alpha; T.V[e] = vn; }
-        if (S.in.itn == 0) { T.H[e] = vn; T.HBAR[e] = 0.0; T.XIN[e] = 0.0; }
-        else {
-          double ho = T.H[e];
-          double hb = T.HBAR[e] * S.in.cf_hbar + ho;
-          T.HBAR[e] = hb;
-          double xn = T.XIN[e] + S.in.cf_x * hb;
-          T.XIN[e] = xn;
-          T.H[e] = ho * S.in.cf_h + vn;
-          red[0] += xn * xn;
-        }
-        T.W[e] = T.D[e] * vn;
-      } break;
-      case EW_STEP1: {
-        double ph = -T.XIN[e];
-        T.PH[e] = ph;
-        double x = X[i], p = T.D[e] * ph, xp = x + p;
-        red[6] = fmin(red[6], fmin(xp - lb, ub - xp));
-        red[5] += p * T.G[e];
-        red[7] = fmax(red[7], -step_to_bound(x, p, lb, ub));
-      } break;
-      case EW_STEP2: {
-        double ph = T.PH[e], x = X[i], d = T.D[e];
-        double p = d * ph;
-        double st = step_to_bound(x, p, lb, ub);
-        double rh = (st == S.p_stride && p != 0.0) ? -ph : ph;
-        T.RH[e] = rh;
-        T.PH[e] = ph * S.p_stride;
-        double xb = x + p * S.p_stride, r = d * rh;
-        red[7] = fmax(red[7], -step_to_bound(xb, r, lb, ub));
-        T.W[e] = r;
-      } break;
-      case EW_LOAD_PH: T.W[e] = T.D[e] * T.PH[e]; break;
-      case EW_DOTS: {
-        double ph = T.PH[e], rh = T.RH[e], dh = T.DH[e], gh = T.D[e] * T.G[e];
-        red[0] += rh * dh * rh; red[1] += gh * rh; red[2] += ph * dh * rh; red[3] += gh * ph; red[4] += ph * dh * ph;
-      } break;
-      case EW_AG: {
-        double d = T.D[e], g = T.G[e], gh = d * g, agh = -gh, ag = d * agh;
-        red[0] += agh * T.DH[e] * agh; red[1] += gh * agh;
-        red[7] = fmax(red[7], -step_to_bound(X[i], ag, lb, ub));
-        T.W[e] = ag;
-      } break;
-      case EW_MKSTEP: {
-        double d = T.D[e];
-        double s2 = d * (S.coef_p * T.PH[e] + S.coef_r * T.RH[e] - S.coef_ag * (d * T.G[e]));
-        T.STEP[e] = s2; T.W[e] = s2; red[0] += s2 * T.G[e];
-      } break;
-      case EW_XUPD: {
-        double x = X[i];
-        if (S.cost_change >= 0) {
-          x = x + T.STEP[e];
-          if (x <= lb) x = nextafter(lb, ub);
-          if (x >= ub) x = nextafter(ub, lb);
-          if (x < lb || x > ub) x = 0.5 * (lb + ub);
-          X[i] = x;
-        }
-        T.W[e] = x;
-      } break;
-      case EW_FINAL: B.xs[e] = (float)X[i]; break;
-    }
-  }
-  if (op == EW_LOAD_PH || op == EW_XUPD || op == EW_FINAL) return;
-  trf_store_partials(T, c, blockIdx.x, red, shd);
-}
-
-__global__ void __launch_bounds__(HB2_BLOCK) k_trf_start_apply(BD B, TD T) {
-  const int c = blockIdx.y;
-  const TrfState& S = T.st[c];
-  if (!S.active) return;
-  double* X = B.x + (size_t)c * B.npad;
-  const double lb = S.lb, ub = S.ub, d = ub - lb;
-  for (int i = blockIdx.x * HB2_BLOCK * 4 + threadIdx.x, qq = 0; qq < 4; ++qq, i += HB2_BLOCK) {
-    if (i >= B.npad || (i % B.L3P) >= B.L3) continue;
+  if constexpr (OP == EW_START) {
     double y = X[i];
-    double t = fmod(y - lb, 2 * d);
-    if (t < 0) t += 2 * d;
-    double x = lb + fmin(t, 2 * d - t);
+    red[6] = fmin(red[6], y); red[7] = fmax(red[7], y);
+  } else if constexpr (OP == EW_START_APPLY) {
+    const double y = X[i], dd = ub - lb;
+    double t = fmod(y - lb, 2 * dd);
+    if (t < 0) t += 2 * dd;
+    double x = lb + fmin(t, 2 * dd - t);
     double ld = x - lb, udist = ub - x;
     double lth = 0.1 * fmax(1.0, fabs(lb)), uth = 0.1 * fmax(1.0, fabs(ub));
     bool la = ld <= fmin(udist, lth), ua = udist <= fmin(ld, uth);
@@ -459,47 +355,151 @@
     if (ua) x = ub - 0.1 * fmax(1.0, fabs(ub));
     if (x < lb || x > ub) x = 0.5 * (lb + ub);
     X[i] = x;
-    T.W[(size_t)c * B.npad + i] = x;
-  }
-}
-
-enum { MW_RESID = 0, MW_INNER_U, MW_DOTS3, MW_DOT_YY };
-__global__ void __launch_bounds__(HB2_BLOCK) k_trf_mw(BD B, TD T, int op) {
+    T.W[e] = x;
+  } else if constexpr (OP == EW_PREP) {
+    double x = X[i], g = T.G[e], v = 1.0, dv = 0.0;
+    if (g < 0) { v = ub - x; dv = -1.0; }
+    if (g > 0) { v = x - lb; dv = 1.0; }
+    const double d = sqrt(v), dh = g * dv;
+    T.D[e] = d; T.DH[e] = dh;
+    red[7] = fmax(red[7], fabs(g * v));
+    const double gh = d * g;
+    T.UN[e] = 0.0; T.V[e] = gh; red[0] += gh * gh;
+    const double agh = -gh, ag = d * agh;
+    red[1] += agh * dh * agh; red[2] += gh * agh;
+    red[6] = fmin(red[6], step_to_bound(x, ag, lb, ub));
+  } else if constexpr (OP == EW_INNER_V) {
+    double vt = (T.D[e] * T.W[e] + sqrt(T.DH[e]) * T.UN[e]) * S.in.inv_beta - S.in.beta * T.V[e];
+    T.V[e] = vt; red[0] += vt * vt;
+  } else if constexpr (OP == EW_INNER_UPD) {
+    double vn = T.V[e];
+    if (S.in.itn == 0 || !S.in.skip_adj) { vn *= S.in.inv_alpha; T.V[e] = vn; }
+    if (S.in.itn == 0) { T.H[e] = vn; T.HBAR[e] = 0.0; T.XIN[e] = 0.0; }
+    else {
+      double ho = T.H[e];
+      double hb = T.HBAR[e] * S.in.cf_hbar + ho;
+      T.HBAR[e] = hb;
+      double xn = T.XIN[e] + S.in.cf_x * hb;
+      T.XIN[e] = xn;
+      T.H[e] = ho * S.in.cf_h + vn;
+      red[0] += xn * xn;
+    }
+    T.W[e] = T.D[e] * vn;
+  } else if constexpr (OP == EW_STEP1) {
+    double ph = -T.XIN[e];
+    T.PH[e] = ph;
+    double x = X[i], p = T.D[e] * ph, xp = x + p;
+    red[6] = fmin(red[6], fmin(xp - lb, ub - xp));
+    red[5] += p * T.G[e];
+    red[7] = fmax(red[7], -step_to_bound(x, p, lb, ub));
+  } else if constexpr (OP == EW_STEP2) {
+    const double ph = T.PH[e], d = T.D[e];
+    if (S.full_step) { T.W2[e] = d * ph; return; }
+    const double x = X[i], p = d * ph;
+    const double st = step_to_bound(x, p, lb, ub);
+    const double rh = (st == S.p_stride && p != 0.0) ? -ph : ph;
+    const double phs = ph * S.p_stride;
+    T.RH[e] = rh; T.PH[e] = phs;
+    const double xb = x + p * S.p_stride, r = d * rh;
+    red[7] = fmax(red[7], -step_to_bound(xb, r, lb, ub));
+    T.W[e] = r; T.W2[e] = d * phs;
+    const double dh = T.DH[e], gh = d * T.G[e];
+    red[0] += rh * dh * rh; red[1] += gh * rh; red[2] += phs * dh * rh; red[3] += gh * phs; red[4] += phs * dh * phs;
+    T.AG[e] = d * -gh;
+  } else if constexpr (OP == EW_XUPD) {
+    double x = X[i];
+    if (S.cost_change >= 0) {
+      x = x + trf_step(S, T, e);
+      if (x <= lb) x = nextafter(lb, ub);
+      if (x >= ub) x = nextafter(ub, lb);
+      if (x < lb || x > ub) x = 0.5 * (lb + ub);
+      X[i] = x;
+    }
+    T.W[e] = x;
+  } else if constexpr (OP == EW_FINAL) {
+    B.xs[e] = (float)X[i];
+  } else if constexpr (OP == NM_INNER_U) {
+    double un = sqrt(T.DH[e]) * T.V[e] - S.in.alpha * (T.UN[e] * S.in.inv_beta);
+    T.UN[e] = un; red[0] += un * un;
+  } else if constexpr (OP == NM_STEP) {
+    red[1] += trf_step(S, T, e) * T.G[e];
+  }
+}
+
+template <int OP>
+__device__ __forceinline__ void trf_m_elem(const BD& B, const TD& T, const TrfState& S, int c, long long r, size_t e,
+                                           double (&red)[TRF_NRED]) {
+  if constexpr (OP == MW_RESID) {
+    double bb = r < B.cand_mdata[c] ? (double)B.b[e] : 0.0;
+    double res = T.Y[e] - bb;
+    T.R[e] = res; T.UM[e] = res; red[0] += res * res;
+  } else if constexpr (OP == NM_INNER_U) {
+    double un = T.Y[e] - S.in.alpha * (T.UM[e] * S.in.inv_beta);
+    T.UM[e] = un; red[0] += un * un;
+  } else if constexpr (OP == MW_DOTS) {
+    double v1 = T.Y[e], u1 = T.YP[e], a = T.YAG[e];
+    red[0] += v1 * v1; red[1] += u1 * v1; red[2] += u1 * u1; red[3] += a * a;
+  } else if constexpr (OP == NM_STEP) {
+    double v = 0.0;
+    if (S.coef_p != 0.0) v += S.coef_p * T.YP[e];
+    if (S.coef_r != 0.0) v += S.coef_r * T.Y[e];
+    if (S.coef_ag != 0.0) v += S.coef_ag * T.YAG[e];
+    red[0] += v * v;
+  }
+}
+
+template <int OP>
+__global__ void __launch_bounds__(HB2_BLOCK) k_trf_pass(BD B, TD T) {
   const int c = blockIdx.y;
-  __shared__ double shd[HB2_BLOCK / 32];
   const TrfState& S = T.st[c];
-  bool act = op == MW_INNER_U ? trf_gate(S, 1) : (op == MW_DOTS3 ? trf_gate(S, 2) : trf_gate(S, 0));
-  if (!act) return;
-  const long long m = (long long)B.cand_mdata[c] + B.cand_msym[c];
-  const size_t o = (size_t)B.cand_uoff[c];
-  double red[TRF_NRED] = {0, 0, 0, 0, 0, 0, INFINITY, -INFINITY};
-  for (long long r = (long long)blockIdx.x * HB2_BLOCK * 4 + threadIdx.x, qq = 0; qq < 4; ++qq, r += HB2_BLOCK) {
-    if (r >= m) continue;
-    const size_t e = o + r;
-    switch (op) {
-      case MW_RESID: {
-        double bb = r < B.cand_mdata[c] ? (double)B.b[e] : 0.0;
-        double res = T.Y[e] - bb;
-        T.R[e] = res; T.UM[e] = res; red[0] += res * res;
-      } break;
-      case MW_INNER_U: {
-        double un = T.Y[e] - S.in.alpha * (T.UM[e] * S.in.inv_beta);
-        T.UM[e] = un; red[0] += un * un;
-      } break;
-      case MW_DOTS3: {
-        double v1 = T.Y[e], u1 = T.Y2[e];
-        red[0] += v1 * v1; red[1] += u1 * v1; red[2] += u1 * u1;
-      } break;
-      case MW_DOT_YY: { double v = T.Y[e]; red[0] += v * v; } break;
-    }
-  }
-  trf_store_partials(T, c, blockIdx.x, red, shd);
+  if (!trf_pass_active(S, OP)) return;
+  double red[TRF_NRED];
+#pragma unroll
+  for (int k = 0; k < TRF_NRED; ++k) red[k] = trf_identity(k);
+  if (trf_has_n(OP) && (!trf_has_m(OP) || (int)blockIdx.x < T.gn)) {
+    const size_t o = (size_t)c * B.npad;
+    double* X = B.x + o;
+    const int i0 = blockIdx.x * TRF_SPAN + threadIdx.x;
+#pragma unroll 4
+    for (int k = 0; k < TRF_EPT; ++k) {
+      const int i = i0 + k * HB2_BLOCK;
+      if (i >= B.npad || (i % B.L3P) >= B.L3) continue;
+      trf_n_elem<OP>(B, T, S, X, i, o + i, red);
+    }
+  } else if (trf_has_m(OP)) {
+    const long long m = (long long)B.cand_mdata[c] + B.cand_msym[c];
+    const size_t o = (size_t)B.cand_uoff[c];
+    const long long r0 = (long long)(blockIdx.x - (trf_has_n(OP) ? T.gn : 0)) * TRF_SPAN + threadIdx.x;
+#pragma unroll 4
+    for (int k = 0; k < TRF_EPT; ++k) {
+      const long long r = r0 + (long long)k * HB2_BLOCK;
+      if (r >= m) continue;
+      trf_m_elem<OP>(B, T, S, c, r, o + r, red);
+    }
+  }
+  constexpr unsigned mask = trf_mask(OP);
+  if constexpr (mask != 0) {
+    __shared__ double shd[TRF_NRED][HB2_BLOCK / 32];
+    trf_block_reduce(red, mask, shd);
+    if (threadIdx.x == 0) {
+      double* dst = T.red + ((size_t)c * T.red_slots + blockIdx.x) * TRF_NRED;
+#pragma unroll
+      for (int k = 0; k < TRF_NRED; ++k)
+        if (mask >> k & 1u) dst[k] = red[k];
+    }
+  }
 }
 
 enum {
-  SC_START = 0, SC_RESID0, SC_PREP, SC_INNER_INIT, SC_INNER_BETA, SC_INNER_ROT, SC_INNER_TEST, SC_STEP1, SC_STEP2,
-  SC_SAVE_M, SC_QUAD, SC_SAVE_AG, SC_AG, SC_SAVE_SG, SC_CC, SC_RESID
+  SC_START = 0, SC_RESID0, SC_PREP, SC_INNER_BETA, SC_INNER_ROT, SC_INNER_TEST, SC_STEP1, SC_STEP2, SC_SELECT, SC_CC,
+  SC_RESID
 };
+__device__ __forceinline__ bool trf_scal_active(const TrfState& S, int op) {
+  if (op == SC_START) return S.needed != 0;
+  if (op == SC_INNER_BETA || op == SC_INNER_ROT || op == SC_INNER_TEST) return trf_gate(S, 1);
+  if (op == SC_STEP2 || op == SC_SELECT) return trf_gate(S, 2);
+  return trf_gate(S, 0);
+}
 __device__ __forceinline__ void min_quadratic_1d(double a, double b, double lo, double hi, double c, double& t, double& y) {
   double tt[3] = {lo, hi, 0};
   int n = 2;
@@ -513,14 +513,7 @@
     if (yy < y) { y = yy; t = tt[k]; }
   }
 }
-__global__ void k_trf_scal(BD B, TD T, int op, double eps, int lsmr_maxiter, int max_iter) {
-  const int c = blockIdx.x * blockDim.x + threadIdx.x;
-  if (c >= B.nc) return;
-  TrfState& S = T.st[c];
-  if (op == SC_START) { if (!S.needed) return; }
-  else if (op == SC_INNER_BETA || op == SC_INNER_ROT || op == SC_INNER_TEST) { if (!trf_gate(S, 1)) return; }
-  else if (op == SC_STEP2 || op == SC_SAVE_M || op == SC_QUAD || op == SC_SAVE_AG || op == SC_AG) { if (!trf_gate(S, 2)) return; }
-  else if (!trf_gate(S, 0)) return;
+__device__ void trf_scalar(const TD& T, TrfState& S, int op, double eps, int lsmr_maxiter, int max_iter) {
   const double* r = S.acc;
   switch (op) {
     case SC_START: {
@@ -540,16 +533,12 @@
       double eta = 1e-2 * fmin(0.5, S.g_norm);
       S.lsmr_tol = fmax(eps, fmin(0.1, eta * S.g_norm));
       S.theta = 1 - fmin(0.005, S.g_norm);
-      S.in.beta = sqrt(2 * S.cost);
-      S.in.inv_beta = S.in.beta > 0 ? 1.0 / S.in.beta : 0.0;
-      S.in.itn = 0; S.in.active = 1; S.in.skip_adj = 0; S.in.alpha = 0; S.full_step = 0;
-    } break;
-    case SC_INNER_INIT: {
-      double nv = sqrt(r[0]);
-      double beta = S.in.beta;
+      S.full_step = 0;
+      const double beta = sqrt(2 * S.cost), nv = sqrt(r[0]);
       lsmr64_init_(S.in, nv * (beta > 0 ? 1.0 / beta : 0.0), beta);
       S.in.inv_alpha = nv > 0 ? 1.0 / nv : 1.0;
       if (S.in.active) atomicAdd(T.ninner, 1);
+      S.ag_n0 = r[1]; S.ag_n1 = r[2]; S.ag_min = r[6];
     } break;
     case SC_INNER_BETA: {
       S.in.beta = sqrt(r[0]);
@@ -571,20 +560,19 @@
       double rsu = -r[7];
       S.r_stride_l = (1 - S.theta) * rsu;
       S.r_stride_u = rsu * S.theta;
-    } break;
-    case SC_SAVE_M: S.m0 = r[0]; S.m1 = r[1]; S.m2 = r[2]; break;
-    case SC_QUAD: {
-      double a = 0.5 * (S.m0 + r[0]);
-      double b = r[1] + S.m1 + r[2];
-      double cc = 0.5 * S.m2 + r[3] + 0.5 * r[4];
+      for (int k = 0; k < 5; ++k) S.qn[k] = r[k];
+    } break;
+    case SC_SELECT: {
+      const double* q = S.qn;
+      const double m0 = r[0], m1 = r[1], m2 = r[2];
+      double a = 0.5 * (m0 + q[0]);
+      double b = q[1] + m1 + q[2];
+      double cc = 0.5 * m2 + q[3] + 0.5 * q[4];
       if (S.r_stride_u > 0) min_quadratic_1d(a, b, S.r_stride_l, S.r_stride_u, cc, S.r_stride, S.r_value);
       else { S.r_value = INFINITY; S.r_stride = 0; }
       double th = S.theta;
-      S.p_value = 0.5 * (th * th * S.m2 + th * th * r[4]) + th * r[3];
-    } break;
-    case SC_SAVE_AG: S.ag_n0 = r[0]; S.ag_n1 = r[1]; S.ag_min = -r[7]; break;
-    case SC_AG: {
-      double a = 0.5 * (r[0] + S.ag_n0), b = S.ag_n1;
+      S.p_value = 0.5 * (th * th * m2 + th * th * q[4]) + th * q[3];
+      a = 0.5 * (r[3] + S.ag_n0); b = S.ag_n1;
       double ag_value;
       min_quadratic_1d(a, b, 0.0, S.ag_min * S.theta, 0.0, S.ag_stride, ag_value);
       S.ag_value = ag_value;
@@ -592,9 +580,8 @@
       else if (S.r_value < S.p_value && S.r_value < ag_value) { S.coef_p = 1.0; S.coef_r = S.r_stride; S.coef_ag = 0; }
       else { S.coef_p = 0; S.coef_r = 0; S.coef_ag = S.ag_stride; }
     } break;
-    case SC_SAVE_SG: S.step_g = r[0]; break;
     case SC_CC: {
-      S.cost_change = -(0.5 * r[0] + S.step_g);
+      S.cost_change = -(0.5 * r[0] + r[1]);
       if (S.nit <= 24) {
         double* t = S.trace[S.nit - 1];
         t[2] = S.in.itn;
@@ -608,3 +595,27 @@
     } break;
   }
 }
+
+__global__ void __launch_bounds__(HB2_BLOCK) k_trf_reduce(BD B, TD T, int nslots, unsigned mask, int op, double eps,
+                                                          int lsmr_maxiter, int max_iter) {
+  const int c = blockIdx.x;
+  __shared__ double shd[TRF_NRED][HB2_BLOCK / 32];
+  TrfState& S = T.st[c];
+  if (!trf_scal_active(S, op)) return;
+  double v[TRF_NRED];
+#pragma unroll
+  for (int k = 0; k < TRF_NRED; ++k) v[k] = trf_identity(k);
+  for (int s2 = threadIdx.x; s2 < nslots; s2 += HB2_BLOCK) {
+    const double* p = T.red + ((size_t)c * T.red_slots + s2) * TRF_NRED;
+#pragma unroll
+    for (int k = 0; k < TRF_NRED; ++k)
+      if (mask >> k & 1u) v[k] = trf_combine(k, v[k], p[k]);
+  }
+  trf_block_reduce(v, mask, shd);
+  if (threadIdx.x == 0) {
+#pragma unroll
+    for (int k = 0; k < TRF_NRED; ++k)
+      if (mask >> k & 1u) S.acc[k] = v[k];
+    trf_scalar(T, S, op, eps, lsmr_maxiter, max_iter);
+  }
+}
diff --git a/profiles/trf_breakdown.py b/profiles/trf_breakdown.py
--- /dev/null
+++ b/profiles/trf_breakdown.py
@@ -0,0 +1,150 @@
+import argparse
+import json
+import os
+import re
+import subprocess
+import sys
+
+ap = argparse.ArgumentParser()
+ap.add_argument("--repo", default=os.path.dirname(os.path.dirname(os.path.abspath(__file__))))
+ap.add_argument("--chunk", type=int, default=0, help="index into bench.job_chunks (default 0)")
+ap.add_argument("--label", default="this")
+ap.add_argument("--out", default="")
+args = ap.parse_args()
+sys.path.insert(0, os.path.abspath(args.repo))
+
+import numpy as np
+import torch
+from torch.profiler import ProfilerActivity, profile
+
+import bench
+from helicon_b200 import _lib
+from helicon_b200.engine import Batch, Problem
+
+CLASSES = ("fwd64", "fwd64_sym", "adj64", "elementwise", "mspace", "reduce_scalar")
+MSPACE_OPS = None
+
+
+def mspace_ops(repo):
+    src = open(os.path.join(repo, "helicon_b200", "csrc", "hb2_trf.cuh")).read()
+    m = re.search(r"enum \{\s*EW_START = 0,(.*?)\};", src, re.S)
+    if m is None or "k_trf_pass" not in src:
+        return set()
+    names = ["EW_START"] + re.findall(r"^\s*(\w+),?\s*(?://.*)?$", m.group(1), re.M)
+    return {i for i, n in enumerate(names) if n.startswith("MW_")}
+
+
+def kernel_class(name):
+    if "double" in name or "TD" in name:
+        if re.search(r"\bk_fwd64_sym\b", name):
+            return "fwd64_sym"
+        if re.search(r"\bk_(fwd_band|fwd_band_reduce|fwd64_data|fwd_tie|fwd_csr|fwd_bil|fwd_lsym)\b", name) and "double" in name:
+            return "fwd64"
+        if re.search(r"\bk_(adj_tile|adj64|adj_tie|adj_csc|adj_bil|adj_bil_tile|bil_unblend|adj_lsym)\b", name) and (
+                "double" in name or "k_adj64" in name):
+            return "adj64"
+    if re.search(r"\bk_trf_(reduce|scal)\b", name):
+        return "reduce_scalar"
+    if re.search(r"\bk_trf_mw\b", name):
+        return "mspace"
+    m = re.search(r"\bk_trf_pass<(\d+)>", name)
+    if m:
+        return "mspace" if int(m.group(1)) in MSPACE_OPS else "elementwise"
+    if re.search(r"\bk_trf_(ew|start_apply)\b", name):
+        return "elementwise"
+    return None
+
+
+def main():
+    global MSPACE_OPS
+    MSPACE_OPS = mspace_ops(os.path.abspath(args.repo))
+    cfg = bench.CONFIGS["cfg2"]
+    img = bench.config_image(cfg)
+    probs = {}
+
+    def problem(key):
+        if key not in probs:
+            D2, L2, D3, D3i, s, L3 = key
+            probs[key] = Problem(img, s, D2, L2, D3, D3i / 2, D3 // 2 - 1)
+        return probs[key]
+
+    chunks, _ = bench.job_chunks(cfg, args.chunk + 1, cfg["batch"], -1, lambda key: problem(key).ndisk)
+    key, tasks = chunks[args.chunk][0], chunks[args.chunk][1]
+    specs = [t.spec for t in tasks]
+
+    def solve():
+        b = Batch(problem(key), key[5], specs)
+        res = b.solve()
+        torch.cuda.synchronize()
+        return b, res
+
+    b, _ = solve()
+    b.close()
+    with profile(activities=[ProfilerActivity.CUDA]) as prof:
+        b, res = solve()
+    tm = np.zeros(16, dtype=np.float64)
+    _lib.check(_lib.load().hb2_batch_timing(b._h, _lib.ptr(tm)))
+    traces = [b.trf_trace(c) for c in range(b.nc)]
+    b.close()
+    for p in probs.values():
+        p.close()
+
+    ms, n = dict.fromkeys(CLASSES, 0.0), dict.fromkeys(CLASSES, 0)
+    for ev in prof.key_averages():
+        k = kernel_class(ev.key)
+        if k is None or ev.device_type != torch.autograd.DeviceType.CUDA:
+            continue
+        t = getattr(ev, "device_time_total", None)
+        if t is None:
+            t = ev.cuda_time_total
+        ms[k] += t / 1e3
+        n[k] += ev.count
+    trf_nit = res["trf_nit"].astype(int)
+    outer = int(tm[13])
+    total = sum(ms.values())
+    kinds = np.zeros(4, dtype=int)
+    inner, fwd_alg, adj_alg, n_it = 0.0, 0.0, 0.0, 0
+    split = bool(MSPACE_OPS)
+    for tr, nit, status in traces:
+        for row in tr:
+            if row[2] == 0 and row[0] == 0:
+                continue
+            kind, k_in = int(row[3]), float(row[2])
+            kinds[kind] += 1
+            inner += k_in
+            n_it += 1
+            if split:
+                fwd_alg += k_in + (1 if kind == 0 else 3) + 1
+                adj_alg += k_in + 1
+            else:
+                fwd_alg += k_in + (0 if kind == 0 else 3) + 2
+                adj_alg += k_in + 2
+    sm = torch.cuda.get_device_properties(0)
+    try:
+        q = subprocess.run(["nvidia-smi", "--query-gpu=name,power.limit,clocks.max.sm", "--format=csv,noheader"],
+                           capture_output=True, text=True, timeout=30).stdout.strip()
+    except Exception as e:
+        q = f"nvidia-smi unavailable: {e}"
+    out = dict(
+        tree=args.label, card=sm.name, nvidia_smi=q, chunk=args.chunk, candidates=int(b.nc),
+        trf_phase_ms_event=round(float(tm[1]), 2), trf_kernel_ms=round(total, 2),
+        kernel_ms={k: round(v, 2) for k, v in ms.items()}, launches={k: n[k] for k in CLASSES},
+        lockstep_outer_iterations=outer,
+        per_outer_iteration={k: round(n[k] / max(1, outer), 2) for k in CLASSES},
+        sum_trf_nit=int(trf_nit.sum()), mean_trf_nit=round(float(trf_nit.mean()), 3),
+        us_per_candidate_trf_iteration=round(1e3 * total / max(1, int(trf_nit.sum())), 1),
+        candidate_outer_iterations=n_it, mean_inner_iterations=round(inner / max(1, n_it), 3),
+        forwards_per_candidate_outer_iteration=round(fwd_alg / max(1, n_it), 3),
+        adjoints_per_candidate_outer_iteration=round(adj_alg / max(1, n_it), 3),
+        step_kinds=dict(full=int(kinds[0]), p=int(kinds[1]), r=int(kinds[2]), ag=int(kinds[3])),
+        trf_nit=trf_nit.tolist(),
+    )
+    print(json.dumps(out))
+    if args.out:
+        data = json.load(open(args.out)) if os.path.exists(args.out) else {}
+        data[args.label] = out
+        json.dump(data, open(args.out, "w"), indent=1)
+
+
+if __name__ == "__main__":
+    main()
```

New measurement: 60.89, median of 6. +11.8%, better.
